# junka/ffpic

Measured on AMD Instinct MI355X. Metric: Mpixels/s decoded (dequant+IDCT+YUV->BGRA), 4K JPEG batch, higher is better.
Workload: dtype int16 -> int32 -> u8; 1 GPU; C3: 256 x 3840x2160 4:2:0 JPEG coefficient grids per GPU; images_total=256, images_this_rank=256, coded_size=3840x2160, subsampling=4:2:0, parallelism=image ranges over 1 GPU(s), no data-path collective, batch_close=one GPU: stream sync + own record, batch_complete=True

## Files before the change

ffpic_amd/csrc/ffhip_entropy.c:

```c
#include "ffpic_hip.h"
#include "ffhip_entropy_internal.h"

#include <pthread.h>
#include <stdio.h>
#include <stdlib.h>
#include <string.h>

static const uint8_t k_zigzag[64] = {0,  1,  8,  16, 9,  2,  3,  10, 17, 24, 32, 25, 18, 11, 4,  5,
                                     12, 19, 26, 33, 40, 48, 41, 34, 27, 20, 13, 6,  7,  14, 21, 28,
                                     35, 42, 49, 56, 57, 50, 43, 36, 29, 22, 15, 23, 30, 37, 44, 51,
                                     58, 59, 52, 45, 38, 31, 39, 46, 53, 60, 61, 54, 47, 55, 62, 63};

static int huff_build(struct huff *h, const uint8_t counts[16], const uint8_t *vals, int nvals)
{
    memset(h, 0, sizeof *h);
    int code = 0, k = 0;
    memcpy(h->vals, vals, (size_t)nvals);
    for (int len = 1; len <= 16; len++) {
        h->valptr[len] = k;
        h->mincode[len] = code;
        for (int i = 0; i < counts[len - 1]; i++, k++, code++) {
            if (k >= nvals) return -1;
            if (code >= (1 << len)) return -1;
            if (len <= LOOK) {
                int first = code << (LOOK - len), n = 1 << (LOOK - len);
                for (int j = 0; j < n; j++) h->look[first + j] = (uint16_t)((len << 8) | vals[k]);
            }
        }
        h->maxcode[len] = counts[len - 1] ? code - 1 : -1;
        code <<= 1;
    }
    h->maxcode[17] = 0x7fffffff;
    h->present = 1;
    for (int i = 0; i < (1 << LOOK); i++) {
        const unsigned e = h->look[i];
        const int len = (int)(e >> 8), run = (int)((e >> 4) & 15), mag = (int)(e & 15);
        if (!e || !mag || len + mag > LOOK) continue;
        int k = ((i << len) & ((1 << LOOK) - 1)) >> (LOOK - mag);
        if (k < (1 << (mag - 1))) k -= (1 << mag) - 1;
        if (k >= -128 && k <= 127) h->fast[i] = (int16_t)((k * 256) + (run * 16) + len + mag);
    }
    return 0;
}

struct bits {
    const uint8_t *p, *end;
    uint64_t acc;
    int n;
    int marker;
    int dry;
};

static inline void bits_fill(struct bits *b)
{
    if (!b->marker && b->end - b->p >= 8 && b->n <= 56) {
        uint64_t w;
        memcpy(&w, b->p, 8);
        w = __builtin_bswap64(w);
        const uint64_t x = ~w;
        if (!((x - 0x0101010101010101ULL) & ~x & 0x8080808080808080ULL)) {
            const int nb = (64 - b->n) >> 3;
            b->acc = nb == 8 ? w : (b->acc << (8 * nb)) | (w >> (64 - 8 * nb));
            b->p += nb;
            b->n += 8 * nb;
            return;
        }
    }
    while (b->n <= 56) {
        unsigned c = 0;
        int real = 0;
        if (!b->marker && b->p < b->end) {
            c = *b->p;
            if (c == 0xFF) {
                if (b->p + 1 < b->end && b->p[1] == 0) { b->p += 2; real = 1; }
                else { b->marker = 1; c = 0; }
            } else { b->p++; real = 1; }
        }
        b->dry += !real;
        b->acc = (b->acc << 8) | c;
        b->n += 8;
    }
}
static inline int bits_get(struct bits *b, int k)
{
    if (k == 0) return 0;
    if (b->n < k) bits_fill(b);
    b->n -= k;
    return (int)((b->acc >> b->n) & ((1u << k) - 1));
}
static inline int huff_decode(struct bits *b, const struct huff *h)
{
    if (b->n < 16) bits_fill(b);
    unsigned peek = (unsigned)((b->acc >> (b->n - LOOK)) & ((1u << LOOK) - 1));
    unsigned e = h->look[peek];
    if (e) { b->n -= (int)(e >> 8); return (int)(e & 0xff); }
    int code = (int)peek, len = LOOK;
    while (code > h->maxcode[len]) {
        if (++len > 16) return -1;
        code = (int)((b->acc >> (b->n - len)) & ((1u << len) - 1));
    }
    b->n -= len;
    return h->vals[(h->valptr[len] + code - h->mincode[len]) & 255];
}
static inline int extend(int v, int t) { return (t && v < (1 << (t - 1))) ? v - (1 << t) + 1 : v; }

static int parse_headers(const uint8_t *f, size_t len, struct jpeg_hdr *j)
{
    memset(j, 0, sizeof *j);
    for (int t = 0; t < 4; t++)
        for (int i = 0; i < 64; i++) j->quant[t][i] = 1;
    if (len < 4 || f[0] != 0xFF || f[1] != 0xD8) return FFHIP_EINVAL;
    size_t p = 2;
    int have_sof = 0;
    while (p + 4 <= len) {
        if (f[p] != 0xFF) return FFHIP_EINVAL;
        while (p < len && f[p] == 0xFF) p++;
        if (p >= len) return FFHIP_EINVAL;
        const int m = f[p++];
        if (m == 0xD9) return FFHIP_EINVAL;
        if (m == 0x01 || (m >= 0xD0 && m <= 0xD7)) continue;
        if (p + 2 > len) return FFHIP_EINVAL;
        const size_t L = ((size_t)f[p] << 8) | f[p + 1];
        if (L < 2 || p + L > len) return FFHIP_EINVAL;
        const uint8_t *s = f + p + 2;
        const size_t sl = L - 2;
        p += L;
        if (m == 0xDB) {
            size_t i = 0;
            while (i < sl) {
                const int prec = s[i] >> 4, id = s[i] & 15;
                i++;
                if (id > 3 || i + (size_t)64 * (prec + 1) > sl) return FFHIP_EINVAL;
                for (int k = 0; k < 64; k++, i += prec + 1)
                    j->quant[id][k_zigzag[k]] = prec ? (uint16_t)((s[i] << 8) | s[i + 1]) : s[i];
            }
        } else if (m == 0xC4) {
            size_t i = 0;
            while (i + 17 <= sl) {
                const int tc = s[i] >> 4, th = s[i] & 15;
                int n = 0;
                for (int k = 0; k < 16; k++) n += s[i + 1 + k];
                if (tc > 1 || th > 3 || n > 256 || i + 17 + (size_t)n > sl) return FFHIP_EINVAL;
                if (huff_build(tc ? &j->ac[th] : &j->dc[th], s + i + 1, s + i + 17, n)) return FFHIP_EINVAL;
                i += 17 + (size_t)n;
            }
        } else if (m == 0xC0 || m == 0xC1) {
            if (sl < 6 || s[0] != 8) return FFHIP_EINVAL;
            j->height = (s[1] << 8) | s[2];
            j->width = (s[3] << 8) | s[4];
            j->ncomp = s[5];
            if ((j->ncomp != 1 && j->ncomp != 3) || sl < (size_t)(6 + 3 * j->ncomp)) return FFHIP_EINVAL;
            if (j->width == 0 || j->height == 0) return FFHIP_EINVAL;
            for (int c = 0; c < j->ncomp; c++) {
                j->cid[c] = s[6 + 3 * c];
                j->h[c] = s[7 + 3 * c] >> 4;
                j->v[c] = s[7 + 3 * c] & 15;
                j->tq[c] = s[8 + 3 * c];
                if (j->tq[c] > 3) return FFHIP_EINVAL;
            }
            have_sof = 1;
        } else if (m == 0xC2 || (m >= 0xC5 && m <= 0xCF && m != 0xC8 && m != 0xCC)) {
            return FFHIP_EINVAL;
        } else if (m == 0xDD) {
            if (sl < 2) return FFHIP_EINVAL;
            j->restart = (s[0] << 8) | s[1];
        } else if (m == 0xDA) {
            if (!have_sof || sl < 1 || s[0] != j->ncomp || sl < (size_t)(4 + 2 * j->ncomp)) return FFHIP_EINVAL;
            for (int k = 0; k < j->ncomp; k++) {
                int c;
                for (c = 0; c < j->ncomp && j->cid[c] != s[1 + 2 * k]; c++) {}
                if (c == j->ncomp) return FFHIP_EINVAL;
                j->td[c] = s[2 + 2 * k] >> 4;
                j->ta[c] = s[2 + 2 * k] & 15;
                if (j->td[c] > 3 || j->ta[c] > 3 || !j->dc[j->td[c]].present || !j->ac[j->ta[c]].present) return FFHIP_EINVAL;
            }
            const uint8_t *t = s + 1 + 2 * j->ncomp;
            if (t[0] != 0 || t[1] != 63 || t[2] != 0) return FFHIP_EINVAL;
            j->scan = f + p;
            j->scan_len = len - p;
            break;
        }
    }
    if (!j->scan) return FFHIP_EINVAL;
    if (j->ncomp == 1) { j->h[0] = j->v[0] = 1; }
    if (j->h[0] < 1 || j->v[0] < 1 || j->h[0] * j->v[0] > 4) return FFHIP_EINVAL;
    for (int c = 1; c < j->ncomp; c++)
        if (j->h[c] != 1 || j->v[c] != 1) return FFHIP_EINVAL;
    return FFHIP_OK;
}

int ffhip_jpeg_parse(const uint8_t *file, size_t len, struct jpeg_hdr *j) { return parse_headers(file, len, j); }
int ffhip_jpeg_probe_restart(const uint8_t *file, size_t len)
{
    struct jpeg_hdr *j = malloc(sizeof *j);
    if (!j) return -1;
    const int r = parse_headers(file, len, j) ? -1 : j->restart;
    free(j);
    return r;
}

int ffhip_jpeg_probe(const uint8_t *file, size_t len, ffhip_jpeg_geom *geom, int *width, int *height)
{
    struct jpeg_hdr *j = malloc(sizeof *j);
    if (!j) return FFHIP_ENOMEM;
    int rc = file && geom ? parse_headers(file, len, j) : FFHIP_EINVAL;
    if (rc == FFHIP_OK) {
        geom->ncomp = j->ncomp;
        geom->h = j->h[0];
        geom->v = j->v[0];
        geom->mcu_cols = (j->width + 8 * j->h[0] - 1) / (8 * j->h[0]);
        geom->mcu_rows = (j->height + 8 * j->v[0] - 1) / (8 * j->v[0]);
        for (int c = 0; c < 3; c++) geom->qt_id[c] = c < j->ncomp ? j->tq[c] : 0;
        if (width) *width = j->width;
        if (height) *height = j->height;
    }
    free(j);
    return rc;
}

static int decode_mcus(const struct jpeg_hdr *j, int16_t *const planes[3], struct bits *b, long mcu, long count)
{
    int pred[3] = {0, 0, 0};
    for (int c = 0; c < j->ncomp; c++) {
        const size_t per = (size_t)j->h[c] * j->v[c] * 64;
        memset(planes[c] + (size_t)mcu * per, 0, (size_t)count * per * sizeof(int16_t));
    }
    for (const long end = mcu + count; mcu < end; mcu++) {
        for (int c = 0; c < j->ncomp; c++) {
            const struct huff *hd = &j->dc[j->td[c]], *ha = &j->ac[j->ta[c]];
            const int nb = j->h[c] * j->v[c];
            for (int k = 0; k < nb; k++) {
                int16_t *blk = planes[c] + (mcu * nb + k) * 64;
                const int t = huff_decode(b, hd);
                if (t < 0 || t > 11) return FFHIP_EINVAL;
                pred[c] += extend(bits_get(b, t), t);
                blk[0] = (int16_t)pred[c];
                for (int i = 1; i < 64;) {
                    if (b->n < 16) bits_fill(b);
                    const int f = ha->fast[(b->acc >> (b->n - LOOK)) & ((1u << LOOK) - 1)];
                    if (f) {
                        i += (f >> 4) & 15;
                        if (i > 63) return FFHIP_EINVAL;
                        b->n -= f & 15;
                        blk[k_zigzag[i++]] = (int16_t)(f >> 8);
                        continue;
                    }
                    const int rs = huff_decode(b, ha);
                    if (rs < 0) return FFHIP_EINVAL;
                    const int r = rs >> 4, s = rs & 15;
                    if (s == 0) {
                        if (r == 15) { i += 16; continue; }
                        break;
                    }
                    i += r;
                    if (i > 63) return FFHIP_EINVAL;
                    blk[k_zigzag[i]] = (int16_t)extend(bits_get(b, s), s);
                    i++;
                }
            }
        }
    }
    if (b->dry * 8 > b->n) return FFHIP_EINVAL;
    return FFHIP_OK;
}

struct interval_job {
    const struct jpeg_hdr *j;
    int16_t *planes[3];
    const size_t *seg;
    long n_seg, mcus, first, last;
    int rc;
};
static void *interval_worker(void *arg)
{
    struct interval_job *w = arg;
    w->rc = FFHIP_OK;
    for (long i = w->first; i < w->last && w->rc == FFHIP_OK; i++) {
        const uint8_t *p = w->j->scan + w->seg[i];
        const uint8_t *e = i + 1 < w->n_seg ? w->j->scan + w->seg[i + 1] - 2 : w->j->scan + w->j->scan_len;
        struct bits b = {p, e, 0, 0, 0, 0};
        const long mcu = i * w->j->restart, left = w->mcus - mcu;
        w->rc = decode_mcus(w->j, w->planes, &b, mcu, left < w->j->restart ? left : w->j->restart);
    }
    return NULL;
}

int ffhip_jpeg_entropy_decode_mt(const uint8_t *file, size_t len, const ffhip_jpeg_geom *expect, int16_t *coef_y,
                                 int16_t *coef_u, int16_t *coef_v, uint16_t *quant , int n_threads)
{
    struct jpeg_hdr *j = malloc(sizeof *j);
    if (!j) return FFHIP_ENOMEM;
    int rc = file && coef_y && quant ? parse_headers(file, len, j) : FFHIP_EINVAL;
    if (rc) { free(j); return rc; }
    const int mcu_cols = (j->width + 8 * j->h[0] - 1) / (8 * j->h[0]), mcu_rows = (j->height + 8 * j->v[0] - 1) / (8 * j->v[0]);
    if (expect && (expect->mcu_cols != mcu_cols || expect->mcu_rows != mcu_rows || expect->ncomp != j->ncomp ||
                   expect->h != j->h[0] || expect->v != j->v[0])) { free(j); return FFHIP_EINVAL; }
    if (j->ncomp == 3 && (!coef_u || !coef_v)) { free(j); return FFHIP_EINVAL; }
    memcpy(quant, j->quant, sizeof j->quant);
    const long mcus = (long)mcu_cols * mcu_rows;
    struct interval_job base = {j, {coef_y, coef_u, coef_v}, NULL, 1, mcus, 0, 1, FFHIP_OK};
    if (!j->restart) {
        struct bits b = {j->scan, j->scan + j->scan_len, 0, 0, 0, 0};
        rc = decode_mcus(j, base.planes, &b, 0, mcus);
        free(j);
        return rc;
    }
    const long n_seg = (mcus + j->restart - 1) / j->restart;
    size_t *seg = malloc((size_t)n_seg * sizeof *seg);
    if (!seg) { free(j); return FFHIP_ENOMEM; }
    long found = 1;
    seg[0] = 0;
    for (size_t q = 0; q + 1 < j->scan_len && found < n_seg; q++)
        if (j->scan[q] == 0xFF && j->scan[q + 1] >= 0xD0 && j->scan[q + 1] <= 0xD7) { seg[found++] = q + 2; q++; }
    if (found != n_seg) { free(seg); free(j); return FFHIP_EINVAL; }
    base.seg = seg;
    base.n_seg = n_seg;
    if (n_threads < 1) n_threads = 1;
    if (n_threads > n_seg) n_threads = (int)n_seg;
    if (n_threads > 64) n_threads = 64;
    struct interval_job jobs[64];
    pthread_t tid[64];
    int started[64] = {0};
    for (int t = 0; t < n_threads; t++) {
        jobs[t] = base;
        jobs[t].first = n_seg * t / n_threads;
        jobs[t].last = n_seg * (t + 1) / n_threads;
        if (t) started[t] = pthread_create(&tid[t], NULL, interval_worker, &jobs[t]) == 0;
    }
    interval_worker(&jobs[0]);
    rc = jobs[0].rc;
    for (int t = 1; t < n_threads; t++) {
        if (started[t]) pthread_join(tid[t], NULL);
        else interval_worker(&jobs[t]);
        if (rc == FFHIP_OK) rc = jobs[t].rc;
    }
    free(seg);
    free(j);
    return rc;
}

int ffhip_jpeg_entropy_decode(const uint8_t *file, size_t len, const ffhip_jpeg_geom *expect, int16_t *coef_y,
                              int16_t *coef_u, int16_t *coef_v, uint16_t *quant )
{
    return ffhip_jpeg_entropy_decode_mt(file, len, expect, coef_y, coef_u, coef_v, quant, 1);
}

struct batch_job {
    const uint8_t *const *files;
    const size_t *lens;
    const ffhip_jpeg_geom *g;
    int first, last;
    int16_t *y, *u, *v;
    uint16_t *quant;
    int *status;
};
static void blank_picture(int16_t *y, int16_t *u, int16_t *v, uint16_t *quant, size_t yb, size_t cb)
{
    memset(y, 0, yb * sizeof(int16_t));
    if (u) memset(u, 0, cb * sizeof(int16_t));
    if (v) memset(v, 0, cb * sizeof(int16_t));
    for (int i = 0; i < 256; i++) quant[i] = 1;
}
static void *batch_worker(void *arg)
{
    struct batch_job *jb = arg;
    const size_t mcus = (size_t)jb->g->mcu_cols * jb->g->mcu_rows, yb = mcus * jb->g->h * jb->g->v * 64, cb = mcus * 64;
    for (int i = jb->first; i < jb->last; i++) {
        jb->status[i] = ffhip_jpeg_entropy_decode(jb->files[i], jb->lens[i], jb->g, jb->y + i * yb, jb->u ? jb->u + i * cb : NULL,
                                                  jb->v ? jb->v + i * cb : NULL, jb->quant + (size_t)i * 256);
        if (jb->status[i]) blank_picture(jb->y + i * yb, jb->u ? jb->u + i * cb : NULL, jb->v ? jb->v + i * cb : NULL, jb->quant + (size_t)i * 256, yb, cb);
    }
    return NULL;
}

int ffhip_jpeg_entropy_batch(const uint8_t *const *files, const size_t *lens, int n, int n_threads,
                             const ffhip_jpeg_geom *geom, int16_t *coef_y, int16_t *coef_u, int16_t *coef_v,
                             uint16_t *quant, int *status)
{
    if (n < 0 || !geom || (n > 0 && (!files || !lens || !coef_y || !quant || !status))) return FFHIP_EINVAL;
    if (n == 0) return FFHIP_OK;
    if (n_threads < 1) n_threads = 1;
    if (n_threads >= 2 * n) {
        const size_t mcus = (size_t)geom->mcu_cols * geom->mcu_rows, yb = mcus * geom->h * geom->v * 64, cb = mcus * 64;
        int first_err = FFHIP_OK;
        for (int i = 0; i < n; i++) {
            status[i] = ffhip_jpeg_entropy_decode_mt(files[i], lens[i], geom, coef_y + (size_t)i * yb, coef_u ? coef_u + (size_t)i * cb : NULL,
                                                     coef_v ? coef_v + (size_t)i * cb : NULL, quant + (size_t)i * 256, n_threads);
            if (status[i]) blank_picture(coef_y + (size_t)i * yb, coef_u ? coef_u + (size_t)i * cb : NULL, coef_v ? coef_v + (size_t)i * cb : NULL, quant + (size_t)i * 256, yb, cb);
            if (status[i] && !first_err) first_err = status[i];
        }
        return first_err;
    }
    if (n_threads > n) n_threads = n;
    if (n_threads > 256) n_threads = 256;
    struct batch_job jobs[256];
    pthread_t tid[256];
    int started[256] = {0};
    for (int t = 0; t < n_threads; t++) {
        jobs[t] = (struct batch_job){files, lens, geom, (int)((long)n * t / n_threads), (int)((long)n * (t + 1) / n_threads),
                                     coef_y, coef_u, coef_v, quant, status};
        if (t) started[t] = pthread_create(&tid[t], NULL, batch_worker, &jobs[t]) == 0;
    }
    batch_worker(&jobs[0]);
    for (int t = 1; t < n_threads; t++) {
        if (started[t]) pthread_join(tid[t], NULL);
        else batch_worker(&jobs[t]);
    }
    for (int i = 0; i < n; i++)
        if (status[i]) return status[i];
    return FFHIP_OK;
}

int ffhip_bmp_write(const char *path, const uint8_t *bgra, int width, int height, int64_t pitch)
{
    if (!path || !bgra || width <= 0 || height <= 0 || pitch < (int64_t)width * 4) return FFHIP_EINVAL;
    FILE *f = fopen(path, "wb");
    if (!f) return FFHIP_EIO;
    uint8_t h[54] = {0};
    const uint32_t img = (uint32_t)width * (uint32_t)height * 4u, size = 54u + img;
    const int32_t neg_h = -height;
#define PUT32(o, v) do { uint32_t v__ = (uint32_t)(v); h[o] = v__ & 255; h[(o) + 1] = (v__ >> 8) & 255; h[(o) + 2] = (v__ >> 16) & 255; h[(o) + 3] = v__ >> 24; } while (0)
    h[0] = 'B'; h[1] = 'M';
    PUT32(2, size); PUT32(10, 0x36); PUT32(14, 0x28); PUT32(18, width); PUT32(22, neg_h);
    h[26] = 1; h[28] = 32;
    PUT32(34, img); PUT32(38, 0x60); PUT32(42, 0x60); PUT32(46, 2);
#undef PUT32
    int ok = fwrite(h, 54, 1, f) == 1;
    for (int y = 0; ok && y < height; y++) ok = fwrite(bgra + (size_t)y * (size_t)pitch, (size_t)width * 4, 1, f) == 1;
    ok = (fclose(f) == 0) && ok;
    return ok ? FFHIP_OK : FFHIP_EIO;
}
```

ffpic_amd/csrc/ffhip_entropy_internal.h:

```cpp
#ifndef FFHIP_ENTROPY_INTERNAL_H
#define FFHIP_ENTROPY_INTERNAL_H

#include <stddef.h>
#include <stdint.h>

#ifdef __cplusplus
extern "C" {
#endif

#define LOOK 9
struct huff {
    uint16_t look[1 << LOOK];
    int32_t maxcode[18];
    int32_t valptr[17], mincode[17];
    uint8_t vals[256];
    int present;
    int16_t fast[1 << LOOK];
};

struct jpeg_hdr {
    int width, height, ncomp, restart;
    int h[3], v[3], tq[3], td[3], ta[3], cid[3];
    uint16_t quant[4][64];
    struct huff dc[4], ac[4];
    const uint8_t *scan;
    size_t scan_len;
};

int ffhip_jpeg_parse(const uint8_t *file, size_t len, struct jpeg_hdr *j);
int ffhip_jpeg_probe_restart(const uint8_t *file, size_t len);

#ifdef __cplusplus
}
#endif
#endif
```

ffpic_amd/csrc/ffhip_huff_gpu.hip:

```cpp
#include "ffhip_internal.h"
#include <chrono>
#if defined(__SSE2__)
#include <emmintrin.h>
#endif
#include "ffhip_entropy_internal.h"

#include <stddef.h>
#include <stdlib.h>
#include <string.h>

#include <vector>
#include <memory>
#include <new>

struct HuffImage {
    uint32_t scan_off, scan_len;
    uint32_t seg_base, n_seg;
    uint32_t restart, mcus;
    uint32_t mcu_base;
    uint32_t ncomp, nb[3];
    uint32_t tab_dc[3], tab_ac[3];
};

struct HuffArgs {
    const uint8_t *scan;
    const struct huff *tabs;
    const uint16_t *lut;
    const HuffImage *images;
    const uint32_t *seg;
    const u32x2 *work;
    int16_t *plane[3];
    int *status;
    uint32_t n_work;
};

__device__ static const uint8_t kZigzag[64] = {0,  1,  8,  16, 9,  2,  3,  10, 17, 24, 32, 25, 18, 11, 4,  5,
                                               12, 19, 26, 33, 40, 48, 41, 34, 27, 20, 13, 6,  7,  14, 21, 28,
                                               35, 42, 49, 56, 57, 50, 43, 36, 29, 22, 15, 23, 30, 37, 44, 51,
                                               58, 59, 52, 45, 38, 31, 39, 46, 53, 60, 61, 54, 47, 55, 62, 63};

#define LUT_GROUPS 8
#define LUT_NO_CODE 0x5000u
#define LUT_WORDS (512 + 128 * LUT_GROUPS)

template <int RING_DW, int REFILL_EVERY>
__global__ __launch_bounds__(256) void k_jpeg_huff(HuffArgs a)
{
    __shared__ uint8_t zz[64];
    __shared__ uint16_t lt[6][LUT_WORDS];
    __shared__ uint32_t ring[4][RING_DW][64];
    const uint32_t lane = threadIdx.x & 63, wv = threadIdx.x >> 6;
    if (threadIdx.x < 64) zz[threadIdx.x] = kZigzag[threadIdx.x];
    const uint32_t gid0 = blockIdx.x * 256;
    const uint32_t img0 = a.work[gid0].x;
    const HuffImage im0 = a.images[img0];
    for (int t = 0; t < 3; t++) {
        const u32x4 *sd = (const u32x4 *)(a.lut + (size_t)im0.tab_dc[t] * LUT_WORDS), *sa = (const u32x4 *)(a.lut + (size_t)im0.tab_ac[t] * LUT_WORDS);
        for (int i = (int)threadIdx.x; i < LUT_WORDS / 8; i += 256) {
            ((u32x4 *)lt[t])[i] = sd[i];
            ((u32x4 *)lt[3 + t])[i] = sa[i];
        }
    }
    __syncthreads();
    const uint32_t gid = gid0 + wv * 64 + lane;
    const bool exists = gid < a.n_work;
    const u32x2 w = a.work[exists ? gid : gid0];
    const HuffImage im = a.images[w.x];
    bool in_lds = true;
    for (int t = 0; t < 3; t++) in_lds = in_lds && im.tab_dc[t] == im0.tab_dc[t] && im.tab_ac[t] == im0.tab_ac[t];
    const uint32_t start = im.scan_off + a.seg[im.seg_base + w.y];
    const u32x4 *src = (const u32x4 *)(a.scan + (start & ~15u));
    uint32_t rd = (start & 15u) >> 2, wr = 0;
    const uint32_t dw_end = (im.scan_off + a.seg[im.seg_base + w.y + 1] - (start & ~15u)) >> 2;
    uint32_t mcu = w.y * im.restart;
    const uint32_t mcu_end = mcu + im.restart < im.mcus ? mcu + im.restart : im.mcus;
    __shared__ uint32_t slotrec[4][8][64];
    __shared__ int predv[4][3][64];
    __shared__ unsigned long long planeb[4][3][64];
    uint32_t nbt = 0;
#pragma unroll
    for (int c = 0; c < 3; c++) {
        const unsigned long long pb = a.plane[c] ? (unsigned long long)(uintptr_t)(a.plane[c] + (size_t)im.mcu_base * im.nb[c] * 64) : 0ull;
        planeb[wv][c][lane] = pb;
        predv[wv][c][lane] = 0;
        for (uint32_t kb0 = 0; kb0 < im.nb[c] && nbt < 8; kb0++)
            slotrec[wv][nbt++][lane] = (uint32_t)c | (kb0 << 2) | (im.nb[c] << 5) | ((im.tab_dc[c] & 0xfffu) << 8) | ((im.tab_ac[c] & 0xfffu) << 20);
    }
    unsigned long long acc = 0;
    int n = 0;
    bool active = exists && mcu < mcu_end, bad = false;
    uint32_t slot = 0, k = 0, rec = slotrec[wv][0][lane];
    int16_t *blk = (int16_t *)(uintptr_t)planeb[wv][0][lane] + (size_t)mcu * im.nb[0] * 64;
    int pred_cur = 0;
    auto refill = [&]() {
        while (__builtin_amdgcn_ballot_w64(wr + 4 <= rd + RING_DW)) {
            if (wr + 4 <= rd + RING_DW) {
                u32x4 v = {0u, 0u, 0u, 0u};
                if (wr < dw_end) v = src[wr >> 2];
#pragma unroll
                for (int j = 0; j < 4; j++) ring[wv][(wr + j) & (RING_DW - 1)][lane] = wr + j < dw_end ? v[j] : 0u;
                wr += 4;
            }
        }
    };
    refill();
    for (int i = 0; i < 2; i++) {
        const uint32_t d = ring[wv][rd & (RING_DW - 1)][lane];
        acc = (acc << 32) | __builtin_bswap32(d);
        rd++;
    }
    n = 64;
    for (uint32_t iter = 1; __builtin_amdgcn_ballot_w64(active); iter++) {
        if ((iter & (REFILL_EVERY - 1)) == 0) refill();
        const uint32_t nextdw = ring[wv][rd & (RING_DW - 1)][lane];
        if (active) {
            const bool dc = k == 0;
            const uint32_t c = rec & 3u;
            const unsigned top = (unsigned)(acc >> 32);
            const unsigned peek = top >> (32 - LOOK);
            const uint32_t tix = dc ? (rec >> 8) & 0xfffu : rec >> 20;
            unsigned e;
            if (in_lds) {
                const uint16_t *l = lt[dc ? c : 3 + c];
                e = l[peek];
                if (e & 0x8000u) e = l[512 + ((e & 0xffu) << 7) + ((top >> (32 - 16)) & 127u)];
            } else {
                const uint16_t *l = a.lut + (size_t)tix * LUT_WORDS;
                e = l[peek];
                if (e & 0x8000u) e = l[512 + ((e & 0xffu) << 7) + ((top >> (32 - 16)) & 127u)];
            }
            int sym = (int)(e & 0xff), len = (int)((e >> 8) & 31u);
            bad |= (e & 0x4000u) != 0;
            if (!e) {
                const struct huff *T = a.tabs + tix;
                int code = (int)peek;
                len = LOOK;
                while (len < 17 && code > T->maxcode[len]) {
                    len++;
                    code = (int)(top >> (32 - len));
                }
                if (len > 16) { bad = true; len = 16; }
                sym = T->vals[(T->valptr[len] + code - T->mincode[len]) & 255];
            }
            acc <<= len;
            const int s = dc ? sym : (sym & 15), r = dc ? 0 : (sym >> 4);
            const bool skip = !dc && s == 0;
            k += skip ? (r == 15 ? 16u : 64u) : (uint32_t)r;
            const unsigned vb = (unsigned)((acc >> 33) >> (31 - s));
            acc <<= s;
            n -= len + s;
            const int lim = (1 << s) >> 1;
            int v = (int)vb < lim ? (int)vb - (1 << s) + 1 : (int)vb;
            pred_cur += dc ? v : 0;
            v = dc ? pred_cur : v;
            bad |= (dc && s > 11) || (!skip && k > 63);
            if (!skip && k <= 63) blk[zz[k]] = (int16_t)v;
            k += skip ? 0u : 1u;
            if (k >= 64) {
                k = 0;
                slot++;
                const bool wrap = slot == nbt;
                slot = wrap ? 0u : slot;
                mcu += wrap ? 1u : 0u;
                rec = slotrec[wv][slot][lane];
                const uint32_t c2 = rec & 3u, nbc = (rec >> 5) & 7u, kb = (rec >> 2) & 7u;
                predv[wv][c][lane] = pred_cur;
                pred_cur = predv[wv][c2][lane];
                blk = (int16_t *)(uintptr_t)planeb[wv][c2][lane] + (size_t)(mcu * nbc + kb) * 64;
                if (mcu >= mcu_end) active = false;
            }
            bad |= rd > dw_end + 2;
#ifdef HUFF_DEBUG
            if (rd > dw_end + 2) printf("lane %u img %u seg %u: rd %u lim %u start %u mcu %u/%u k %u n %d\n", gid, w.x, w.y, rd, dw_end, start, mcu, mcu_end, k, n);
#endif
            if (bad) active = false;
            if (n <= 32) {
                acc |= (unsigned long long)__builtin_bswap32(nextdw) << (32 - n);
                n += 32;
                rd++;
            }
        }
    }
    if (bad) a.status[w.x] = FFHIP_EINVAL;
}

namespace {
uint32_t stage_scan(uint8_t *dst, const uint8_t *src, const uint8_t *end, uint32_t *seg, uint32_t n_seg, size_t *clean_len, uint32_t *raw = nullptr)
{
    uint8_t *d = dst;
    uint32_t k = 0;
    seg[0] = 0;
    for (;;) {
#if defined(__SSE2__)
        const __m128i ff = _mm_set1_epi8((char)0xFF);
        while (src + 16 <= end) {
            const __m128i v = _mm_loadu_si128((const __m128i *)src);
            const unsigned m = (unsigned)_mm_movemask_epi8(_mm_cmpeq_epi8(v, ff));
            _mm_storeu_si128((__m128i *)d, v);
            if (m) {
                const int c = __builtin_ctz(m);
                src += c;
                d += c;
                break;
            }
            src += 16;
            d += 16;
        }
#endif
        while (src < end && *src != 0xFF) *d++ = *src++;
        if (src + 1 >= end) break;
        const uint8_t b = src[1];
        if (b == 0) { *d++ = 0xFF; src += 2; continue; }
        if (b < 0xD0 || b > 0xD7 || k + 1 >= n_seg) break;
        {
            const size_t len = (size_t)(d - dst) - seg[k], padded = ((len + 3) & ~(size_t)3) + 4;
            memset(d, 0, padded - len);
            d = dst + seg[k] + padded;
            if (raw) raw[k] = (uint32_t)len;
            seg[++k] = (uint32_t)(d - dst);
            src += 2;
        }
    }
    {
        const size_t len = (size_t)(d - dst) - seg[k], padded = ((len + 3) & ~(size_t)3) + 4;
        memset(d, 0, padded - len);
        d = dst + seg[k] + padded;
        if (raw) raw[k] = (uint32_t)len;
    }
    *clean_len = (size_t)(d - dst);
    return k + 1;
}

void build_lut(const struct huff &h, uint16_t *out)
{
    memset(out, 0, LUT_WORDS * sizeof(uint16_t));
    memcpy(out, h.look, 512 * sizeof(uint16_t));
    int groups = 0;
    bool complete = true;
    for (int len = LOOK + 1; len <= 16; len++) {
        if (h.maxcode[len] < 0) continue;
        for (int code = h.mincode[len]; code <= h.maxcode[len]; code++) {
            const int idx = h.valptr[len] + code - h.mincode[len];
            if (idx < 0 || idx > 255 || code >= (1 << len)) return;
            const int prefix = code >> (len - LOOK);
            if (out[prefix] && !(out[prefix] & 0x8000)) return;
            if (!out[prefix]) {
                if (groups == LUT_GROUPS) { complete = false; continue; }
                out[prefix] = (uint16_t)(0x8000 | groups++);
            }
            const int g = out[prefix] & 0xff;
            const int rest = (code << (16 - len)) & 127, cnt = 1 << (16 - len);
            for (int k = 0; k < cnt; k++) out[512 + 128 * g + rest + k] = (uint16_t)((len << 8) | h.vals[idx]);
        }
    }
    if (complete)
        for (int i = 0; i < 512 + 128 * groups; i++)
            if (!out[i]) out[i] = LUT_NO_CODE;
}
}

extern "C" int ffhip_jpeg_stage_scan_test(uint8_t *dst, const uint8_t *src, size_t len, uint32_t *seg, uint32_t n_seg, size_t *clean_len)
{
    if (!dst || !src || !seg || !clean_len || n_seg == 0) return FFHIP_EINVAL;
    return (int)stage_scan(dst, src, src + len, seg, n_seg, clean_len);
}

extern "C" int ffhip_jpeg_stage_scan_raw_test(uint8_t *dst, const uint8_t *src, size_t len, uint32_t *seg, uint32_t n_seg, size_t *clean_len, uint32_t *raw)
{
    if (!dst || !src || !seg || !clean_len || !raw || n_seg == 0) return FFHIP_EINVAL;
    return (int)stage_scan(dst, src, src + len, seg, n_seg, clean_len, raw);
}
extern "C" int ffhip_jpeg_lut_test(const uint8_t *file, size_t len, int which, uint16_t *out)
{
    if (!file || !out || which < 0 || which > 7) return FFHIP_EINVAL;
    std::unique_ptr<struct jpeg_hdr> j(new (std::nothrow) struct jpeg_hdr);
    if (!j) return FFHIP_ENOMEM;
    if (ffhip_jpeg_parse(file, len, j.get())) return FFHIP_EINVAL;
    const struct huff &h = which < 4 ? j->dc[which] : j->ac[which - 4];
    if (!h.present) return FFHIP_EINVAL;
    build_lut(h, out);
    return FFHIP_OK;
}

static thread_local double g_huff_times[8] = {0, 0, 0, 0, 0, 0, 0, 0};
static uint32_t sync_sub_bits(unsigned long long bits, unsigned long long mcus)
{
    const char *b = FFHIP_ENV("FFHIP_JPEG_SYNC_BITS");
    const long sb = b ? atol(b) : bits <= 1024 * mcus ? 2048 : bits <= 2048 * mcus ? 4096 : 8192;
    return (uint32_t)(sb < 128 ? 128 : sb > 65536 ? 65536 : sb);
}
extern "C" int ffhip_debug_huff_times(double out[8])
{
    if (!out) return FFHIP_EINVAL;
    for (int k = 0; k < 8; k++) out[k] = g_huff_times[k];
    return FFHIP_OK;
}

struct SyncSeg {
    uint32_t pic;
    uint32_t scan_off, clean_len;
    uint32_t raw_len;
    uint32_t mcu0, mcus;
};
struct SyncJob {
    uint8_t *dev;
    size_t o_tabs, o_l12, o_status;
    int n, part;
    void *stream;
    const HuffImage *images;
    const SyncSeg *segs;
    size_t n_segs;
    int16_t *plane[3];
    uint32_t rounds_used;
    uint32_t n_tasks;
    int reran;
    uint32_t rounds;
    uint32_t sub_bits;
};
static int huff_sync_enqueue(SyncJob &job, void *stream, uint32_t **h_cnt);
static int huff_sync_finish(SyncJob &job, void *stream, uint32_t *h_cnt, int *status);

namespace {
typedef std::chrono::steady_clock::time_point HuffTime;
HuffTime huff_now() { return std::chrono::steady_clock::now(); }
long us(HuffTime a, HuffTime b) { return (long)std::chrono::duration_cast<std::chrono::microseconds>(b - a).count(); }
struct HuffLayout { size_t o_tabs, o_l12, o_img, o_seg, o_work, o_status, o_quant, total; };
HuffLayout huff_layout(size_t scan_total, size_t n_tabs, size_t n, size_t seg_total)
{
    HuffLayout L;
    size_t at = scan_total + 16;
    auto take = [&](size_t bytes) { const size_t o = at; at = (at + bytes + 15) & ~(size_t)15; return o; };
    L.o_tabs = take(n_tabs * sizeof(struct huff));
    L.o_l12 = take(n_tabs * LUT_WORDS * 2);
    L.o_img = take(n * sizeof(HuffImage));
    L.o_seg = take((seg_total + n) * 4);
    L.o_work = take(seg_total * 8);
    L.o_status = take(n * 4);
    L.o_quant = take(n * 512);
    L.total = at;
    return L;
}
struct HuffCall {
    const uint8_t *const *files;
    const size_t *lens;
    int n, n_threads;
    const ffhip_jpeg_geom *geom, *geoms;
    int16_t *d_coef_y, *d_coef_u, *d_coef_v;
    uint16_t *d_quant;
    int *status;
    hipStream_t st;
    const FfhipHuffThen *then;
    std::vector<uint32_t> pic_mcus, mcu_base;
    struct jpeg_hdr *hdr;
    std::vector<std::vector<uint32_t>> segs, raws;
    uint32_t sub_bits;
    std::vector<HuffImage> images;
    std::vector<const struct huff *> uniq;
    size_t scan_total, seg_total;
    HuffLayout L;
    uint8_t *stage, *dev;
    hipStream_t up, second;
    hipEvent_t fork, join, *part_ev, time_ev[2];
    std::vector<ffhip_jpeg_item> then_items;
    bool times;
    HuffTime T0, T1, T2, T3, T4;
    long staging_us, tables_us;
};

#define HUFF_TRY(call) do { if ((call) != hipSuccess) return FFHIP_EIO; } while (0)
int huff_first_status(const HuffCall &c) { for (int i = 0; i < c.n; i++) if (c.status[i]) return c.status[i]; return FFHIP_OK; }
int huff_check(HuffCall &c)
{
    const ffhip_jpeg_geom *geom = c.geom;
    if (geom->ncomp == 3 && (!c.d_coef_u || !c.d_coef_v)) return FFHIP_EINVAL;
    c.n_threads = c.n_threads < 1 ? 1 : c.n_threads > 64 ? 64 : c.n_threads;
    if (geom->mcu_cols <= 0 || geom->mcu_rows <= 0 || geom->h < 1 || geom->v < 1 || geom->h * geom->v > 4 ||
        (geom->ncomp != 1 && geom->ncomp != 3)) return FFHIP_EINVAL;
    c.pic_mcus.resize((size_t)c.n);
    c.mcu_base.resize((size_t)c.n + 1);
    size_t sum = 0;
    for (int i = 0; i < c.n; i++) {
        const ffhip_jpeg_geom *gi = c.geoms ? &c.geoms[i] : geom;
        if (c.geoms && (gi->ncomp != geom->ncomp || gi->h != geom->h || gi->v != geom->v || gi->mcu_cols <= 0 || gi->mcu_rows <= 0)) return FFHIP_EINVAL;
        c.pic_mcus[(size_t)i] = (uint32_t)((size_t)gi->mcu_cols * gi->mcu_rows);
        c.mcu_base[(size_t)i] = (uint32_t)sum;
        sum += c.pic_mcus[(size_t)i];
        if (sum > 0xffffffffu) return FFHIP_EINVAL;
    }
    c.mcu_base[(size_t)c.n] = (uint32_t)sum;
    return FFHIP_OK;
}
int huff_parse_headers(HuffCall &c)
{
    c.hdr = ffhip_huff_hdr_records((size_t)c.n);
    if (!c.hdr) return FFHIP_ENOMEM;
    c.segs.resize((size_t)c.n);
    c.raws.resize((size_t)c.n);
    ffhip_parallel_for(c.n, c.n_threads, [&c](int i) {
        struct jpeg_hdr &j = c.hdr[(size_t)i];
        c.status[i] = ffhip_jpeg_parse(c.files[i], c.lens[i], &j);
        if (c.status[i]) return;
        const int mc = (j.width + 8 * j.h[0] - 1) / (8 * j.h[0]), mr = (j.height + 8 * j.v[0] - 1) / (8 * j.v[0]);
        const ffhip_jpeg_geom *gi = c.geoms ? &c.geoms[i] : c.geom;
        const size_t mcus = c.pic_mcus[(size_t)i];
        if (mc != gi->mcu_cols || mr != gi->mcu_rows || j.ncomp != gi->ncomp || j.h[0] != gi->h || j.v[0] != gi->v ||
            j.scan_len > 0x7fffffffu) {
            c.status[i] = FFHIP_EINVAL;
            return;
        }
        if (!j.restart) j.restart = (int)mcus;
        c.segs[(size_t)i].assign((size_t)((mcus + j.restart - 1) / j.restart) + 1, 0u);
        c.raws[(size_t)i].assign(c.segs[(size_t)i].size(), 0u);
    });
    return huff_first_status(c);
}
bool huff_choose_subsequences(HuffCall &c)
{
    const char *sy = FFHIP_ENV("FFHIP_JPEG_SYNC");
    unsigned long long batch_bits = 0, n_int = 0;
    for (int i = 0; i < c.n; i++) batch_bits += 8ull * c.hdr[(size_t)i].scan_len;
    c.sub_bits = sync_sub_bits(batch_bits, (unsigned long long)c.mcu_base[(size_t)c.n]);
    if (sy && (sy[0] == '0' || sy[0] == '1')) return sy[0] == '1';
    for (int i = 0; i < c.n; i++) n_int += c.segs[(size_t)i].size() - 1;
    return batch_bits > 2ull * c.sub_bits * n_int;
}
uint32_t huff_table_id(std::vector<const struct huff *> &uniq, const struct huff *t)
{
    for (size_t u = uniq.size(); u-- > 0;)
        if (uniq[u] == t || !memcmp(&uniq[u]->maxcode, &t->maxcode, offsetof(struct huff, fast) - offsetof(struct huff, maxcode))) return (uint32_t)u;
    uniq.push_back(t);
    return (uint32_t)(uniq.size() - 1);
}
int huff_lay_out(HuffCall &c)
{
    c.images.resize((size_t)c.n);
    c.scan_total = c.seg_total = 0;
    for (int i = 0; i < c.n; i++) {
        const struct jpeg_hdr &j = c.hdr[(size_t)i];
        HuffImage &im = c.images[(size_t)i];
        im.scan_off = (uint32_t)c.scan_total;
        im.scan_len = (uint32_t)j.scan_len;
        im.restart = (uint32_t)j.restart;
        im.mcus = c.pic_mcus[(size_t)i];
        im.mcu_base = c.mcu_base[(size_t)i];
        im.ncomp = (uint32_t)j.ncomp;
        im.seg_base = (uint32_t)c.seg_total;
        im.n_seg = (uint32_t)c.segs[(size_t)i].size() - 1;
        for (int k = 0; k < 3; k++) {
            im.nb[k] = k < j.ncomp ? (uint32_t)(j.h[k] * j.v[k]) : 0;
            im.tab_dc[k] = huff_table_id(c.uniq, &j.dc[k < j.ncomp ? j.td[k] : j.td[0]]);
            im.tab_ac[k] = huff_table_id(c.uniq, &j.ac[k < j.ncomp ? j.ta[k] : j.ta[0]]);
        }
        c.scan_total += (j.scan_len + 8 * (size_t)im.n_seg + 64 + 15) & ~(size_t)15;
        c.seg_total += im.n_seg;
        im.seg_base += (uint32_t)i;
        if (c.scan_total > 0x7fffffffu) return FFHIP_EINVAL;
    }
    if (!ffhip_have_device()) return FFHIP_ENODEV;
    if (c.uniq.size() > 4095) return FFHIP_EINVAL;
    c.L = huff_layout(c.scan_total, c.uniq.size(), (size_t)c.n, c.seg_total);
    c.stage = ffhip_pinned_scratch(SCRATCH_HUFF, c.st, c.L.total + 64);
    if (!c.stage) return FFHIP_ENOMEM;
    c.T2 = huff_now();
    c.dev = (uint8_t *)ffhip_scratch(SCRATCH_HUFF, c.st, (c.L.total + 3) / 4);
    return c.dev ? FFHIP_OK : FFHIP_ENOMEM;
}
int huff_clear_planes(HuffCall &c)
{
    const size_t total_mcus = c.mcu_base[(size_t)c.n], yb = total_mcus * c.geom->h * c.geom->v * 64;
    FFHIP_CHECK(hipMemsetAsync(c.d_coef_y, 0, yb * 2, c.st), FFHIP_EIO);
    if (c.geom->ncomp != 3) return FFHIP_OK;
    FFHIP_CHECK(hipMemsetAsync(c.d_coef_u, 0, total_mcus * 128, c.st), FFHIP_EIO);
    FFHIP_CHECK(hipMemsetAsync(c.d_coef_v, 0, total_mcus * 128, c.st), FFHIP_EIO);
    return FFHIP_OK;
}
void huff_stage_pictures(HuffCall &c, int lo, int hi, bool lists)
{
    ffhip_parallel_for(hi - lo, c.n_threads, [&c, lo, lists](int i_rel) {
        const int i = lo + i_rel;
        const struct jpeg_hdr &j = c.hdr[(size_t)i];
        const HuffImage &im = c.images[(size_t)i];
        uint8_t *dst = c.stage + im.scan_off;
        std::vector<uint32_t> &sgv = c.segs[(size_t)i];
        size_t off = 0;
        if (stage_scan(dst, j.scan, j.scan + j.scan_len, sgv.data(), im.n_seg, &off, c.raws[(size_t)i].data()) != im.n_seg) c.status[i] = FFHIP_EINVAL;
        memset(dst + off, 0, 16);
        sgv[im.n_seg] = (uint32_t)off;
        if (!lists) return;
        uint32_t *sg = (uint32_t *)(c.stage + c.L.o_seg) + im.seg_base;
        u32x2 *wk = (u32x2 *)(c.stage + c.L.o_work) + (im.seg_base - (uint32_t)i);
        for (uint32_t k = 0; k < im.n_seg; k++) {
            sg[k] = sgv[k];
            wk[k].x = (uint32_t)i;
            wk[k].y = k;
        }
        sg[im.n_seg] = (uint32_t)off;
        memcpy(c.stage + c.L.o_quant + (size_t)i * 512, j.quant, 512);
    });
}
int huff_part_lo(const HuffCall &c, int n_parts, int part) { return (int)((long long)c.n * part / n_parts); }
size_t huff_scan_end(const HuffCall &c, int hi) { return hi < c.n ? c.images[(size_t)hi].scan_off : c.scan_total; }

int huff_tail_up(HuffCall &c)
{
    const HuffTime Ta = huff_now();
    memset(c.stage + c.scan_total, 0, 16);
    ffhip_parallel_for((int)c.uniq.size(), c.n_threads, [&c](int u) {
        ((struct huff *)(c.stage + c.L.o_tabs))[u] = *c.uniq[(size_t)u];
        build_lut(*c.uniq[(size_t)u], (uint16_t *)(c.stage + c.L.o_l12) + (size_t)u * LUT_WORDS);
    });
    memcpy(c.stage + c.L.o_img, c.images.data(), c.images.size() * sizeof(HuffImage));
    memset(c.stage + c.L.o_status, 0, (size_t)c.n * 4);
    c.tables_us = us(Ta, huff_now());
    FFHIP_CHECK(hipMemcpyAsync(c.dev + c.scan_total, c.stage + c.scan_total, c.L.total - c.scan_total, hipMemcpyHostToDevice, c.st), FFHIP_EIO);
    FFHIP_CHECK(hipMemcpyAsync(c.d_quant, c.dev + c.L.o_quant, (size_t)c.n * 512, hipMemcpyDeviceToDevice, c.st), FFHIP_EIO);
    return FFHIP_OK;
}
int huff_reconstruct(HuffCall &c, int lo, int hi, void *on, int part)
{
    const FfhipHuffThen *then = c.then;
    if (!then->items) {
        const size_t mcus = c.pic_mcus[0];
        return ffhip_jpeg_recon_batch(c.geom, hi - lo, c.d_coef_y + (size_t)lo * mcus * c.geom->h * c.geom->v * 64, c.d_coef_u ? c.d_coef_u + (size_t)lo * mcus * 64 : nullptr,
                                      c.d_coef_v ? c.d_coef_v + (size_t)lo * mcus * 64 : nullptr, c.d_quant + (size_t)lo * 256, 256,
                                      then->bgra + (int64_t)lo * then->image_stride, then->pitch, then->image_stride, nullptr, 0, on);
    }
    c.then_items.assign(then->items + lo, then->items + hi);
    for (int i = lo; i < hi; i++) jpeg_item_planes(&c.then_items[(size_t)(i - lo)], c.d_coef_y, c.d_coef_u, c.d_coef_v, c.d_quant, c.mcu_base[(size_t)i], (size_t)i);
    return jpeg_recon_items_by_rule(c.then_items.data(), then->rule.at(lo), hi - lo, on, part);
}
int huff_collect(HuffCall &c)
{
    HUFF_TRY(hipMemcpyAsync(c.stage + c.L.o_status, c.dev + c.L.o_status, (size_t)c.n * 4, hipMemcpyDeviceToHost, c.st));
    const HuffTime T5 = huff_now();
    HUFF_TRY(hipStreamSynchronize(c.st));
    const HuffTime T6 = huff_now();
    if (c.times) {
        fprintf(stderr, "huff staging: header parse %ld us, layout %ld us, unstuff + markers (uploads enqueued by parts) %ld us, tables %ld us (%d files, %zu bytes, %d threads)\n", us(c.T0, c.T1), us(c.T1, c.T2), c.staging_us, c.tables_us, c.n, c.L.total, c.n_threads);
        fprintf(stderr, "huff device: enqueue %ld us, wait for uploads + clears + kernel %ld us\n", us(c.T3, T5), us(T5, T6));
    }
    float kms = 0.0f;
    if (hipEventElapsedTime(&kms, c.time_ev[0], c.time_ev[1]) != hipSuccess) { (void)hipGetLastError(); kms = 0.0f; }
    g_huff_times[0] = (double)us(c.T0, c.T1); g_huff_times[1] = (double)us(c.T1, c.T2); g_huff_times[2] = (double)c.staging_us; g_huff_times[3] = (double)c.tables_us;
    g_huff_times[4] = (double)us(c.T4, T5); g_huff_times[5] = (double)us(T5, T6); g_huff_times[6] = (double)kms * 1e3; g_huff_times[7] = (double)us(c.T0, T6);
    memcpy(c.status, c.stage + c.L.o_status, (size_t)c.n * 4);
    return FFHIP_OK;
}
int huff_decode_intervals(HuffCall &c)
{
    const int n_parts = c.n >= 32 ? 4 : 1;
    for (int part = 0; part < n_parts; part++) {
        const int lo = huff_part_lo(c, n_parts, part), hi = huff_part_lo(c, n_parts, part + 1);
        const size_t b0 = huff_scan_end(c, lo), b1 = huff_scan_end(c, hi);
        huff_stage_pictures(c, lo, hi, true);
        HUFF_TRY(hipMemcpyAsync(c.dev + b0, c.stage + b0, b1 - b0, hipMemcpyHostToDevice, c.st));
    }
    if (huff_first_status(c)) return huff_first_status(c);
    c.T3 = huff_now();
    c.staging_us = us(c.T2, c.T3);
    const int rc = huff_tail_up(c);
    if (rc) return rc;
    c.T4 = huff_now();
    HuffArgs a;
    a.scan = c.dev;
    a.tabs = (const struct huff *)(c.dev + c.L.o_tabs);
    a.lut = (const uint16_t *)(c.dev + c.L.o_l12);
    a.images = (const HuffImage *)(c.dev + c.L.o_img);
    a.seg = (const uint32_t *)(c.dev + c.L.o_seg);
    a.work = (const u32x2 *)(c.dev + c.L.o_work);
    a.plane[0] = c.d_coef_y; a.plane[1] = c.d_coef_u; a.plane[2] = c.d_coef_v;
    a.status = (int *)(c.dev + c.L.o_status);
    a.n_work = (uint32_t)c.seg_total;
    (void)hipEventRecord(c.time_ev[0], c.st);
    {
        int cus = 256, device = 0;
        if (hipGetDevice(&device) == hipSuccess) (void)hipDeviceGetAttribute(&cus, hipDeviceAttributeMultiprocessorCount, device);
        const unsigned wgs = (a.n_work + 255) / 256;
        const char *fr = FFHIP_ENV("FFHIP_HUFF_RING");
        if (fr ? atoi(fr) == 16 : wgs > 2u * (unsigned)cus) hipLaunchKernelGGL((k_jpeg_huff<16, 8>), dim3(wgs), dim3(256), 0, c.st, a);
        else hipLaunchKernelGGL((k_jpeg_huff<32, 16>), dim3(wgs), dim3(256), 0, c.st, a);
    }
    HUFF_TRY(hipGetLastError());
    (void)hipEventRecord(c.time_ev[1], c.st);
    if (c.then) {
        const int rrc = huff_reconstruct(c, 0, c.n, c.st, 0);
        if (rrc) return rrc;
    }
    return huff_collect(c);
}
int huff_sync_part_count(const HuffCall &c)
{
    const int by_bytes = (int)((c.scan_total + (70u << 20)) / (140u << 20));
    int n_parts = c.n < 32 || c.scan_total < (16u << 20) ? 1 : by_bytes < 2 ? 2 : by_bytes > FFHIP_HUFF_PARTS ? FFHIP_HUFF_PARTS : by_bytes;
    const char *e = FFHIP_ENV("FFHIP_JPEG_SYNC_PARTS");
    if (e && atoi(e) >= 1) n_parts = atoi(e) > FFHIP_HUFF_PARTS ? FFHIP_HUFF_PARTS : atoi(e);
    return n_parts > c.n ? c.n : n_parts;
}
int huff_sync_job(const HuffCall &c, SyncJob &job, std::vector<SyncSeg> &segs, int part, int lo, int hi)
{
    job.sub_bits = c.sub_bits;
    job.dev = c.dev; job.o_tabs = c.L.o_tabs; job.o_l12 = c.L.o_l12; job.o_status = c.L.o_status + (size_t)lo * 4; job.n = hi - lo; job.part = part;
    job.images = c.images.data() + lo;
    segs.clear();
    for (int i = lo; i < hi; i++) {
        const HuffImage &im = c.images[(size_t)i];
        const std::vector<uint32_t> &sgv = c.segs[(size_t)i];
        if (c.status[i]) return c.status[i];
        for (uint32_t k = 0; k < im.n_seg; k++) {
            SyncSeg sg;
            sg.pic = (uint32_t)(i - lo);
            sg.scan_off = im.scan_off + sgv[k];
            sg.clean_len = sgv[k + 1] - sgv[k];
            sg.raw_len = c.raws[(size_t)i][k];
            sg.mcu0 = (uint32_t)((size_t)(c.mcu_base[(size_t)i] - c.mcu_base[(size_t)lo]) + (size_t)k * im.restart);
            const size_t left = im.mcus - (size_t)k * im.restart;
            sg.mcus = (uint32_t)(left < im.restart ? left : im.restart);
            segs.push_back(sg);
        }
    }
    job.segs = segs.data();
    job.n_segs = segs.size();
    const size_t base = c.mcu_base[(size_t)lo];
    job.plane[0] = c.d_coef_y + base * c.images[0].nb[0] * 64;
    job.plane[1] = c.d_coef_u ? c.d_coef_u + base * c.images[0].nb[1] * 64 : nullptr;
    job.plane[2] = c.d_coef_v ? c.d_coef_v + base * c.images[0].nb[2] * 64 : nullptr;
    return FFHIP_OK;
}
int huff_decode_subsequences(HuffCall &c)
{
    const int n_parts = huff_sync_part_count(c);
    SyncJob jobs[FFHIP_HUFF_PARTS];
    std::vector<SyncSeg> part_segs[FFHIP_HUFF_PARTS];
    uint32_t *h_cnt[FFHIP_HUFF_PARTS];
    for (int i = 0; i < c.n; i++) memcpy(c.stage + c.L.o_quant + (size_t)i * 512, c.hdr[(size_t)i].quant, 512);
    int rc = huff_tail_up(c);
    if (rc) return rc;
    (void)hipEventRecord(c.time_ev[0], c.st);
    const char *ss = FFHIP_ENV("FFHIP_JPEG_SYNC_STREAMS");
    const bool two_streams = n_parts > 1 && !(ss && ss[0] == '1');
    if (two_streams) {
        HUFF_TRY(hipEventRecord(c.fork, c.st));
        HUFF_TRY(hipStreamWaitEvent(c.second, c.fork, 0));
    }
    for (int part = 0; part < n_parts; part++) {
        const int lo = huff_part_lo(c, n_parts, part), hi = huff_part_lo(c, n_parts, part + 1);
        SyncJob &job = jobs[part];
        const size_t b0 = huff_scan_end(c, lo), b1 = huff_scan_end(c, hi);
        huff_stage_pictures(c, lo, hi, false);
        job.stream = two_streams && (part & 1) ? (void *)c.second : c.st;
        HUFF_TRY(hipMemcpyAsync(c.dev + b0, c.stage + b0, b1 - b0, hipMemcpyHostToDevice, c.up));
        HUFF_TRY(hipEventRecord(c.part_ev[part], c.up));
        HUFF_TRY(hipStreamWaitEvent((hipStream_t)job.stream, c.part_ev[part], 0));
        rc = huff_sync_job(c, job, part_segs[part], part, lo, hi);
        if (!rc) rc = huff_sync_enqueue(job, job.stream, &h_cnt[part]);
        if (!rc && c.then) rc = huff_reconstruct(c, lo, hi, job.stream, part);
        if (rc) return rc;
    }
    if (two_streams) {
        HUFF_TRY(hipEventRecord(c.join, c.second));
        HUFF_TRY(hipStreamWaitEvent(c.st, c.join, 0));
    }
    c.T3 = c.T4 = huff_now();
    c.staging_us = us(c.T2, c.T3) - c.tables_us;
    HUFF_TRY(hipGetLastError());
    (void)hipEventRecord(c.time_ev[1], c.st);
    rc = huff_collect(c);
    if (rc) return rc;
    for (int part = 0; part < n_parts; part++) {
        SyncJob &job = jobs[part];
        const int lo = huff_part_lo(c, n_parts, part);
        rc = huff_sync_finish(job, job.stream, h_cnt[part], c.status + lo);
        if (!rc && job.reran && c.then) {
            rc = huff_reconstruct(c, lo, lo + job.n, job.stream, part);
            if (!rc && job.stream != c.st && hipStreamSynchronize((hipStream_t)job.stream) != hipSuccess) rc = FFHIP_EIO;
        }
        if (rc) return rc;
        if (c.times) fprintf(stderr, "huff sync, part %d: %u subsequences of %u bits, %u rounds\n", part, job.n_tasks, job.sub_bits, job.rounds_used);
    }
    return FFHIP_OK;
}
}

int jpeg_entropy_batch_gpu_impl(const uint8_t *const *files, const size_t *lens, int n, int n_threads, const ffhip_jpeg_geom *geom,
                                const ffhip_jpeg_geom *geoms, int16_t *d_coef_y, int16_t *d_coef_u, int16_t *d_coef_v, uint16_t *d_quant,
                                int *status, void *stream, const FfhipHuffThen *then)
{
    if (n < 0 || !geom || (n > 0 && (!files || !lens || !d_coef_y || !d_quant || !status))) return FFHIP_EINVAL;
    if (n == 0) return FFHIP_OK;
    HuffCall c{files, lens, n, n_threads, geom, geoms, d_coef_y, d_coef_u, d_coef_v, d_quant, status, (hipStream_t)stream, then};
    int rc = huff_check(c);
    if (rc) return rc;
    c.times = FFHIP_ENV("FFHIP_HUFF_TIMES") != nullptr;
    c.T0 = huff_now();
    rc = huff_parse_headers(c);
    if (rc) return rc;
    const bool subsequences = huff_choose_subsequences(c);
    c.T1 = huff_now();
    rc = huff_lay_out(c);
    if (rc) return rc;
    rc = huff_clear_planes(c);
    if (rc) return rc;
    FfhipHuffStreams hs;
    if (ffhip_huff_streams_get(&hs) != FFHIP_OK) return FFHIP_EIO;
    c.up = (hipStream_t)hs.up; c.second = (hipStream_t)hs.c2;
    c.part_ev = (hipEvent_t *)hs.part_ev;
    c.fork = (hipEvent_t)hs.fork; c.join = (hipEvent_t)hs.join;
    c.time_ev[0] = (hipEvent_t)hs.time_ev[0]; c.time_ev[1] = (hipEvent_t)hs.time_ev[1];
    rc = subsequences ? huff_decode_subsequences(c) : huff_decode_intervals(c);
    if (rc) {
        (void)hipStreamSynchronize(c.up);
        (void)hipStreamSynchronize(c.second);
        (void)hipStreamSynchronize(c.st);
        (void)hipGetLastError();
        return rc;
    }
    return huff_first_status(c);
}
extern "C" int ffhip_jpeg_entropy_batch_gpu(const uint8_t *const *files, const size_t *lens, int n, int n_threads,
                                            const ffhip_jpeg_geom *geom, int16_t *d_coef_y, int16_t *d_coef_u, int16_t *d_coef_v,
                                            uint16_t *d_quant, int *status, void *stream)
{
    return jpeg_entropy_batch_gpu_impl(files, lens, n, n_threads, geom, nullptr, d_coef_y, d_coef_u, d_coef_v, d_quant, status, stream, nullptr);
}

#define SYNC_ROUNDS_MAX 32

struct SyncImage {
    uint32_t scan_off;
    uint32_t clean_len;
    uint32_t data_bits;
    uint32_t mcus, ncomp, nbt;
    uint32_t nb[3], tab_dc[3], tab_ac[3];
    uint32_t pic, mcu0;
};
struct SyncArgs {
    const uint8_t *scan;
    const struct huff *tabs;
    const uint16_t *lut;
    const SyncImage *images;
    const uint32_t *sub_base;
    unsigned long long *exit_;
    unsigned long long *used;
    u32x4 *sums;
    uint32_t *list;
    uint32_t *seg_of;
    uint32_t *cnt;
    uint32_t *end_pos;
    int16_t *plane[3];
    int *status;
    uint32_t n_tasks, n_images, round, last, sub_bits;
};

__device__ __forceinline__ uint32_t sync_picture_of(const SyncArgs &a, uint32_t t)
{
    return a.seg_of[t];
}
__global__ __launch_bounds__(256) void k_huff_sync_segs(SyncArgs a)
{
    const uint32_t p = blockIdx.x, t1 = a.sub_base[p + 1];
    for (uint32_t t = a.sub_base[p] + threadIdx.x; t < t1; t += 256) a.seg_of[t] = p;
}

#define LIST_THREADS 1024
__global__ __launch_bounds__(LIST_THREADS) void k_huff_sync_list(SyncArgs a)
{
    __shared__ uint32_t wcount[LIST_THREADS / 64], wbase[LIST_THREADS / 64];
    if (a.round >= 3 && a.cnt[a.round - 1] == 0) return;
    const uint32_t t = blockIdx.x * LIST_THREADS + threadIdx.x, lane = threadIdx.x & 63, wv = threadIdx.x >> 6;
    bool stale = false;
    if (t > 0 && t < a.n_tasks) stale = a.seg_of[t - 1] == a.seg_of[t] && a.exit_[t - 1] != a.used[t];
    const unsigned long long m = __builtin_amdgcn_ballot_w64(stale);
    if (lane == 0) wcount[wv] = (uint32_t)__builtin_popcountll(m);
    __syncthreads();
    if (threadIdx.x == 0) {
        uint32_t total = 0;
        for (int w = 0; w < LIST_THREADS / 64; w++) { wbase[w] = total; total += wcount[w]; }
        const uint32_t base = total ? atomicAdd(&a.cnt[a.round], total) : 0u;
        for (int w = 0; w < LIST_THREADS / 64; w++) wbase[w] += base;
    }
    __syncthreads();
    if (stale) a.list[wbase[wv] + (uint32_t)__builtin_popcountll(m & ((1ull << lane) - 1ull))] = t;
}

enum { SPAN_ALL = 0, SPAN_LIST = 1, SPAN_WRITE = 2 };
#define SPAN_THREADS 512
#define WRITE_THREADS 256
template <int MODE, int THREADS>
__global__ __launch_bounds__(THREADS) void k_huff_span(SyncArgs a)
{
    constexpr bool WRITE = MODE == SPAN_WRITE;
    constexpr int RING = 16, REFILL = 4, WAVES = THREADS / 64;
    constexpr uint32_t LUT_BYTES = LUT_WORDS * 2;
    __shared__ uint8_t zz[64];
    __shared__ uint16_t lt[6][LUT_WORDS];
    __shared__ uint32_t ring[WAVES][RING][64];
    __shared__ u32x4 stage[WRITE ? 4 : 1][WRITE ? THREADS : 1];
    const uint32_t lane = threadIdx.x & 63, wv = threadIdx.x >> 6;
    const uint32_t i0 = blockIdx.x * THREADS;
    uint32_t n_here = a.n_tasks;
    if (MODE == SPAN_LIST) {
        n_here = a.cnt[a.round];
        if (i0 >= n_here) return;
    }
    if (WRITE && a.cnt[a.last]) return;
    if (threadIdx.x < 64) zz[threadIdx.x] = kZigzag[threadIdx.x];
    const uint32_t t_first = MODE == SPAN_LIST ? a.list[i0] : i0;
    const uint32_t p0 = sync_picture_of(a, t_first);
    const SyncImage im0 = a.images[p0];
    for (int k2 = 0; k2 < 3; k2++) {
        const u32x4 *sd = (const u32x4 *)(a.lut + (size_t)im0.tab_dc[k2] * LUT_WORDS), *sa = (const u32x4 *)(a.lut + (size_t)im0.tab_ac[k2] * LUT_WORDS);
        for (int i = (int)threadIdx.x; i < LUT_WORDS / 8; i += THREADS) {
            ((u32x4 *)lt[k2])[i] = sd[i];
            ((u32x4 *)lt[3 + k2])[i] = sa[i];
        }
    }
    if (WRITE)
        for (int i = 0; i < 4; i++) stage[i][threadIdx.x] = u32x4{0u, 0u, 0u, 0u};
    uint32_t cpack = 0, kbpack = 0, nbpack = 0;
    {
        uint32_t s = 0;
        for (uint32_t c = 0; c < 3; c++) {
            nbpack |= im0.nb[c] << (3 * c);
            for (uint32_t kb0 = 0; kb0 < im0.nb[c] && s < 8; kb0++, s++) {
                cpack |= c << (2 * s);
                kbpack |= kb0 << (3 * s);
            }
        }
    }
    __syncthreads();
    const uint32_t idx = i0 + threadIdx.x;
    const bool exists = idx < n_here;
    const uint32_t t = exists ? (MODE == SPAN_LIST ? a.list[idx] : idx) : t_first;
    const uint32_t p = exists ? sync_picture_of(a, t) : p0;
    const SyncImage im = a.images[p];
    bool in_lds = true;
    for (int k2 = 0; k2 < 3; k2++) in_lds = in_lds && im.tab_dc[k2] == im0.tab_dc[k2] && im.tab_ac[k2] == im0.tab_ac[k2];
    const uint32_t ti = t - a.sub_base[p];
    const uint32_t total_bits = im.clean_len * 8u;
    uint32_t limit = (ti + 1) * a.sub_bits;
    limit = limit < total_bits ? limit : total_bits;
    unsigned long long entry = 0;
    if (ti > 0) {
        if (WRITE) entry = a.used[t];
        else if (a.round == 0) entry = (unsigned long long)(ti * a.sub_bits);
        else entry = __hip_atomic_load(&a.exit_[t - 1], __ATOMIC_RELAXED, __HIP_MEMORY_SCOPE_AGENT);
    }
    const bool fresh = !WRITE && exists && (a.round == 0 || entry != a.used[t]);
    bool active = WRITE ? exists : fresh;
    uint32_t pos = (uint32_t)entry, slot = (uint32_t)(entry >> 32) & 0xffu, k = (uint32_t)(entry >> 40) & 0xffu;
    if (pos >= limit) active = false;
    const uint32_t nbt = im.nbt, ncomp = im.ncomp;
    u32x4 sm = {0u, 0u, 0u, 0u};
    if (WRITE && exists) sm = a.sums[t];
    slot = slot < nbt ? slot : 0;
    k = k < 64 ? k : 0;
    const uint32_t total_blocks = im.mcus * nbt;
    uint32_t bidx = 0, mcu = 0, blocks = 0;
    bool bad = false;
    if (WRITE) {
        bidx = sm[0];
        mcu = bidx / nbt;
        if (active && bidx < total_blocks && bidx - mcu * nbt != slot) { bad = true; active = false; }
        if (bidx >= total_blocks) active = false;
        mcu += im.mcu0;
    }
    uint32_t c = (cpack >> (2 * slot)) & 3u;
    int pcur, pn1, pn2;
    {
        const int q0 = (int)sm[1], q1 = (int)sm[2], q2 = (int)sm[3];
        pcur = c == 0 ? q0 : c == 1 ? q1 : q2;
        pn1 = c == 0 ? q1 : c == 1 ? q2 : q0;
        pn2 = c == 0 ? q2 : c == 1 ? q0 : q1;
    }
    const uint32_t start = im.scan_off + ((pos >> 5) << 2);
    const u32x4 *src = (const u32x4 *)(a.scan + (start & ~15u));
    uint32_t rd = (start & 15u) >> 2, wr = 0;
    const uint32_t dw_end = (im.scan_off + im.clean_len - (start & ~15u) + 3) >> 2;
    uint32_t *const myring = &ring[wv][0][lane];
    u32x4 pend = {0u, 0u, 0u, 0u};
    bool has_pend = false;
    auto issue = [&]() {
        pend = u32x4{0u, 0u, 0u, 0u};
        if (wr < dw_end) pend = src[wr >> 2];
        has_pend = true;
    };
    auto commit = [&]() {
        uint32_t *d = myring + (wr & (RING - 1)) * 64;
        d[0] = pend[0]; d[64] = pend[1]; d[128] = pend[2]; d[192] = pend[3];
        wr += 4;
        has_pend = false;
    };
    while (__builtin_amdgcn_ballot_w64(wr + 4 <= rd + RING))
        if (wr + 4 <= rd + RING) { issue(); commit(); }
    uint32_t w0 = 0, w1;
    int sh;
    {
        const uint32_t b = pos & 31u;
        if (b) { w0 = __builtin_bswap32(myring[(rd & (RING - 1)) * 64]); rd++; }
        w1 = __builtin_bswap32(myring[(rd & (RING - 1)) * 64]);
        rd++;
        sh = b ? 32 - (int)b : 0;
    }
    int16_t *blk = nullptr;
    auto block_of = [&]() -> int16_t * {
        const uint32_t nbc = (nbpack >> (3 * c)) & 7u, kb = (kbpack >> (3 * slot)) & 7u;
        int16_t *base = c == 0 ? a.plane[0] : c == 1 ? a.plane[1] : a.plane[2];
        return base + (size_t)(mcu * nbc + kb) * 64;
    };
    if (WRITE) blk = block_of();
    uint32_t tb_dc = c * LUT_BYTES;
    uint32_t cmask = 0;
    bool staged = k == 0;
    auto flush_rows = [&]() {
#pragma unroll
        for (int row = 0; row < 4; row++)
            if (cmask & (0xffu << (8 * row))) {
                const u32x4 q = stage[row][threadIdx.x];
                stage[row][threadIdx.x] = u32x4{0u, 0u, 0u, 0u};
                *(u32x4 *)(blk + 8 * row) = q;
            }
        cmask = 0;
    };
    __builtin_amdgcn_s_waitcnt(0x0f70);
    auto run = [&](auto lds_only) {
        constexpr bool LDS_ONLY = decltype(lds_only)::value;
        uint32_t iter = 1;
        while (active) {
            if ((iter & (REFILL - 1)) == 0) {
                if (has_pend) commit();
                if (wr + 4 <= rd + RING) issue();
            }
            iter++;
            const uint32_t nextdw = myring[(rd & (RING - 1)) * 64];
            const uint32_t W = __builtin_amdgcn_alignbit(w0, w1, (uint32_t)sh);
            const bool dc = k == 0;
            unsigned e;
            if (LDS_ONLY || in_lds) {
                const uint16_t *l = (const uint16_t *)((const uint8_t *)lt + tb_dc + (dc ? 0u : 3u * LUT_BYTES));
                e = l[W >> (32 - LOOK)];
                if (e & 0x8000u) e = l[512 + ((e & 0xffu) << 7) + ((W >> 16) & 127u)];
            } else {
                const uint32_t tix = dc ? (c == 0 ? im.tab_dc[0] : c == 1 ? im.tab_dc[1] : im.tab_dc[2]) : (c == 0 ? im.tab_ac[0] : c == 1 ? im.tab_ac[1] : im.tab_ac[2]);
                const uint16_t *l = a.lut + (size_t)tix * LUT_WORDS;
                e = l[W >> (32 - LOOK)];
                if (e & 0x8000u) e = l[512 + ((e & 0xffu) << 7) + ((W >> 16) & 127u)];
            }
            uint32_t sym = e & 0xffu, len = (e >> 8) & 31u;
            if (WRITE) bad |= (e & 0x4000u) != 0;
            if (!e) {
                const uint32_t tix = dc ? (c == 0 ? im.tab_dc[0] : c == 1 ? im.tab_dc[1] : im.tab_dc[2]) : (c == 0 ? im.tab_ac[0] : c == 1 ? im.tab_ac[1] : im.tab_ac[2]);
                const struct huff *T = a.tabs + tix;
                int code = (int)(W >> (32 - LOOK)), ln = LOOK;
                while (ln < 17 && code > T->maxcode[ln]) {
                    ln++;
                    code = (int)(W >> (32 - ln));
                }
                if (ln > 16) { bad = bad || WRITE; ln = 16; code = T->mincode[16]; }
                sym = T->vals[(T->valptr[ln] + code - T->mincode[ln]) & 255];
                len = (uint32_t)ln;
                __builtin_amdgcn_s_waitcnt(0x0f70);
            }
            const uint32_t s = sym & 15u, r = dc ? 0u : sym >> 4;
            const bool skip = !dc && s == 0;
            const uint32_t used = len + s;
            const uint32_t vb = __builtin_amdgcn_ubfe(W, 32u - used, s);
            const uint32_t m1 = (1u << s) - 1u;
            const int v = (vb << 1) > m1 ? (int)vb : (int)vb - (int)m1;
            pcur += dc ? v : 0;
            k += skip ? (r == 15 ? 16u : 64u) : r;
            if (WRITE) {
                bad |= (dc && sym > 11) || (!skip && k > 63);
                if (!skip && k <= 63) {
                    const uint32_t nat = zz[k];
                    const int16_t val = (int16_t)(dc ? pcur : v);
                    if (staged && nat < 32) {
                        ((int16_t *)&stage[nat >> 3][threadIdx.x])[nat & 7u] = val;
                        cmask |= 1u << nat;
                    } else blk[nat] = val;
                }
            }
            k += skip ? 0u : 1u;
            pos += used;
            sh -= (int)used;
            if (sh < 0) {
                w0 = w1;
                w1 = __builtin_bswap32(nextdw);
                sh += 32;
                rd++;
            }
            if (k >= 64) {
                k = 0;
                blocks++;
                slot++;
                const bool wrap = slot == nbt;
                slot = wrap ? 0u : slot;
                const uint32_t c2 = (cpack >> (2 * slot)) & 3u;
                if (c2 != c) { const int q = pcur; pcur = pn1; pn1 = ncomp == 3 ? pn2 : q; pn2 = q; }
                c = c2;
                tb_dc = c * LUT_BYTES;
                if (WRITE) {
                    flush_rows();
                    staged = true;
                    bidx++;
                    mcu += wrap ? 1u : 0u;
                    blk = block_of();
                    if (bidx >= total_blocks) { active = false; a.end_pos[p] = pos; }
                }
            }
            if (pos >= limit || bad) active = false;
        }
    };
    if (__builtin_amdgcn_ballot_w64(!in_lds) == 0) run(std::true_type{});
    else run(std::false_type{});
    if (WRITE) {
        while (cmask) {
            const uint32_t nat = (uint32_t)__builtin_ctz(cmask);
            cmask &= cmask - 1u;
            blk[nat] = ((const int16_t *)&stage[nat >> 3][threadIdx.x])[nat & 7u];
        }
        if (bad) a.status[im.pic] = FFHIP_EINVAL;
        return;
    }
    if (fresh) {
        const int q0 = c == 0 ? pcur : c == 1 ? pn2 : pn1, q1 = c == 0 ? pn1 : c == 1 ? pcur : pn2, q2 = c == 0 ? pn2 : c == 1 ? pn1 : pcur;
        const unsigned long long ex = (unsigned long long)pos | ((unsigned long long)(slot | (k << 8)) << 32);
        __hip_atomic_store(&a.exit_[t], ex, __ATOMIC_RELAXED, __HIP_MEMORY_SCOPE_AGENT);
        a.used[t] = entry;
        u32x4 o;
        o[0] = blocks; o[1] = (uint32_t)q0; o[2] = (uint32_t)q1; o[3] = (uint32_t)q2;
        a.sums[t] = o;
    }
}

__global__ __launch_bounds__(256) void k_huff_sync_scan(SyncArgs a)
{
    __shared__ u32x4 wsum[4];
    const uint32_t p = blockIdx.x;
    if (a.cnt[a.last]) return;
    const SyncImage im = a.images[p];
    const uint32_t t0 = a.sub_base[p], t1 = a.sub_base[p + 1];
    const int lane = threadIdx.x & 63, w = threadIdx.x >> 6;
    u32x4 carry = {0u, 0u, 0u, 0u};
    for (uint32_t base = t0; base < t1; base += 256) {
        const uint32_t t = base + threadIdx.x;
        u32x4 v = {0u, 0u, 0u, 0u};
        if (t < t1) v = a.sums[t];
        u32x4 inc = v;
#pragma unroll
        for (int o = 1; o < 64; o <<= 1) {
#pragma unroll
            for (int q = 0; q < 4; q++) {
                const uint32_t u = (uint32_t)__shfl_up((int)inc[q], o, 64);
                if (lane >= o) inc[q] += u;
            }
        }
        if (lane == 63) wsum[w] = inc;
        __syncthreads();
        u32x4 before = carry, total = {0u, 0u, 0u, 0u};
        for (int q = 0; q < 4; q++) {
            if (q < w) before += wsum[q];
            total += wsum[q];
        }
        if (t < t1) a.sums[t] = before + inc - v;
        carry += total;
        __syncthreads();
    }
    if (threadIdx.x == 0 && carry[0] < im.mcus * im.nbt) a.status[im.pic] = FFHIP_EINVAL;
}

__global__ __launch_bounds__(256) void k_huff_sync_verdict(SyncArgs a)
{
    const uint32_t p = blockIdx.x * 256 + threadIdx.x;
    if (a.cnt[a.last] || p >= a.n_images) return;
    if (a.end_pos[p] > a.images[p].data_bits) a.status[a.images[p].pic] = FFHIP_EINVAL;
}

namespace {
struct SyncLayout { size_t o_img, o_sub, o_cnt, o_end, o_list, o_seg, o_sums, o_exit, o_used, words; };
SyncLayout sync_layout(size_t n, size_t tasks)
{
    SyncLayout L;
    size_t w = 0;
    auto take = [&](size_t words) { const size_t at = w; w += (words + 3) & ~(size_t)3; return at; };
    L.o_img = take(n * sizeof(SyncImage) / 4);
    L.o_sub = take(n + 1);
    L.o_cnt = take(SYNC_ROUNDS_MAX + 3);
    L.o_end = take(n);
    L.o_list = take(tasks);
    L.o_seg = take(tasks);
    L.o_sums = take(4 * tasks);
    L.o_exit = take(2 * tasks);
    L.o_used = take(2 * tasks);
    L.words = w;
    return L;
}
void sync_args(SyncArgs &a, const SyncJob &job, uint32_t *d, const SyncLayout &L)
{
    a.scan = job.dev;
    a.tabs = (const struct huff *)(job.dev + job.o_tabs);
    a.lut = (const uint16_t *)(job.dev + job.o_l12);
    a.images = (const SyncImage *)(d + L.o_img);
    a.sub_base = d + L.o_sub;
    a.exit_ = (unsigned long long *)(d + L.o_exit);
    a.used = (unsigned long long *)(d + L.o_used);
    a.sums = (u32x4 *)(d + L.o_sums);
    a.list = d + L.o_list;
    a.seg_of = d + L.o_seg;
    a.cnt = d + L.o_cnt;
    a.end_pos = d + L.o_end;
    for (int c = 0; c < 3; c++) a.plane[c] = job.plane[c];
    a.status = (int *)(job.dev + job.o_status);
    a.n_tasks = job.n_tasks;
    a.n_images = (uint32_t)job.n_segs;
    a.round = 0;
    a.last = job.rounds + 2;
    a.sub_bits = job.sub_bits;
}
uint32_t sync_tasks_of(uint32_t raw_len, uint32_t sub_bits)
{
    const uint64_t bits = (uint64_t)raw_len * 8;
    return bits ? (uint32_t)((bits + sub_bits - 1) / sub_bits) : 1u;
}
int sync_launch_rounds_and_passes(SyncArgs &a, const SyncJob &job, hipStream_t st)
{
    const unsigned wgs = (job.n_tasks + SPAN_THREADS - 1) / SPAN_THREADS, wgl = (job.n_tasks + LIST_THREADS - 1) / LIST_THREADS;
    for (uint32_t r = 2; r <= job.rounds + 2; r++) {
        a.round = r;
        hipLaunchKernelGGL(k_huff_sync_list, dim3(wgl), dim3(LIST_THREADS), 0, st, a);
        if (r < job.rounds + 2) hipLaunchKernelGGL((k_huff_span<SPAN_LIST, SPAN_THREADS>), dim3(wgs), dim3(SPAN_THREADS), 0, st, a);
    }
    hipLaunchKernelGGL(k_huff_sync_scan, dim3((unsigned)job.n_segs), dim3(256), 0, st, a);
    hipLaunchKernelGGL((k_huff_span<SPAN_WRITE, WRITE_THREADS>), dim3((job.n_tasks + WRITE_THREADS - 1) / WRITE_THREADS), dim3(WRITE_THREADS), 0, st, a);
    hipLaunchKernelGGL(k_huff_sync_verdict, dim3(((unsigned)job.n_segs + 255) / 256), dim3(256), 0, st, a);
    FFHIP_CHECK(hipGetLastError(), FFHIP_EIO);
    return FFHIP_OK;
}
}

static int huff_sync_enqueue(SyncJob &job, void *stream, uint32_t **h_cnt)
{
    static_assert(sizeof(SyncImage) % 4 == 0, "SyncImage is copied by words");
    hipStream_t st = (hipStream_t)stream;
    const size_t n = job.n_segs;
    {
        const char *e = FFHIP_ENV("FFHIP_JPEG_SYNC_ROUNDS");
        const int r = e ? atoi(e) : 10;
        job.rounds = (uint32_t)(r < 1 ? 1 : r > SYNC_ROUNDS_MAX ? SYNC_ROUNDS_MAX : r);
        if (job.sub_bits < 128 || job.sub_bits > 65536) return FFHIP_EINVAL;
    }
    uint64_t tasks = 0;
    for (size_t i = 0; i < n; i++) {
        if (job.segs[i].clean_len >= (1u << 28)) return FFHIP_EINVAL;
        tasks += sync_tasks_of(job.segs[i].raw_len, job.sub_bits);
    }
    if (tasks > 0x7fffff00u || n > 0x7fffff00u) return FFHIP_EINVAL;
    const SyncLayout L = sync_layout(n, (size_t)tasks);
    const size_t head = L.o_list;
    uint8_t *pin = ffhip_pinned_scratch(SCRATCH_HUFF_SYNC + job.part, stream, (head + SYNC_ROUNDS_MAX + 3) * 4);
    uint32_t *d = ffhip_scratch(SCRATCH_HUFF_SYNC + job.part, stream, L.words);
    if (!pin || !d) return FFHIP_ENOMEM;
    uint32_t *h = (uint32_t *)pin;
    SyncImage *si = (SyncImage *)(h + L.o_img);
    uint32_t t = 0;
    for (size_t i = 0; i < n; i++) {
        const SyncSeg &sg = job.segs[i];
        const HuffImage &im = job.images[sg.pic];
        SyncImage &s = si[i];
        s.scan_off = sg.scan_off;
        s.clean_len = sg.clean_len;
        s.data_bits = sg.raw_len * 8u;
        s.mcus = sg.mcus;
        s.pic = sg.pic;
        s.mcu0 = sg.mcu0;
        s.ncomp = im.ncomp;
        s.nbt = 0;
        for (int c = 0; c < 3; c++) { s.nb[c] = im.nb[c]; s.tab_dc[c] = im.tab_dc[c]; s.tab_ac[c] = im.tab_ac[c]; s.nbt += im.nb[c]; }
        if (s.nb[0] != si[0].nb[0] || s.nb[1] != si[0].nb[1] || s.nb[2] != si[0].nb[2]) return FFHIP_EINVAL;
        h[L.o_sub + i] = t;
        t += sync_tasks_of(sg.raw_len, job.sub_bits);
    }
    h[L.o_sub + n] = t;
    job.n_tasks = t;
    memset(h + L.o_cnt, 0, (L.o_end - L.o_cnt) * 4);
    memset(h + L.o_end, 0xff, (L.o_list - L.o_end) * 4);
    FFHIP_CHECK(hipMemcpyAsync(d, h, head * 4, hipMemcpyHostToDevice, st), FFHIP_EIO);
    SyncArgs a;
    sync_args(a, job, d, L);
    const unsigned wgs = (t + SPAN_THREADS - 1) / SPAN_THREADS;
    hipLaunchKernelGGL(k_huff_sync_segs, dim3((unsigned)n), dim3(256), 0, st, a);
    for (uint32_t r = 0; r < 2; r++) {
        a.round = r;
        hipLaunchKernelGGL((k_huff_span<SPAN_ALL, SPAN_THREADS>), dim3(wgs), dim3(SPAN_THREADS), 0, st, a);
    }
    const int rc = sync_launch_rounds_and_passes(a, job, st);
    if (rc) return rc;
    *h_cnt = h + head;
    FFHIP_CHECK(hipMemcpyAsync(*h_cnt, d + L.o_cnt, (SYNC_ROUNDS_MAX + 3) * 4, hipMemcpyDeviceToHost, st), FFHIP_EIO);
    return FFHIP_OK;
}

static int huff_sync_finish(SyncJob &job, void *stream, uint32_t *h_cnt, int *status)
{
    hipStream_t st = (hipStream_t)stream;
    const uint32_t last = job.rounds + 2;
    job.rounds_used = 2;
    job.reran = 0;
    for (uint32_t r = 2; r < last; r++) job.rounds_used += h_cnt[r] ? 1u : 0u;
    if (!h_cnt[last]) return FFHIP_OK;
    const size_t n = job.n_segs;
    const SyncLayout L = sync_layout(n, job.n_tasks);
    uint32_t *d = ffhip_scratch(SCRATCH_HUFF_SYNC + job.part, stream, L.words);
    if (!d) return FFHIP_ENOMEM;
    SyncArgs a;
    sync_args(a, job, d, L);
    uint32_t longest = 0;
    for (size_t i = 0; i < n; i++) {
        const uint32_t ti = sync_tasks_of(job.segs[i].raw_len, job.sub_bits);
        longest = ti > longest ? ti : longest;
    }
    for (uint32_t done = last;; done += job.rounds) {
        if (done > longest + last) return FFHIP_EIO;
        memset(h_cnt, 0, (SYNC_ROUNDS_MAX + 3) * 4);
        FFHIP_CHECK(hipMemcpyAsync(d + L.o_cnt, h_cnt, (SYNC_ROUNDS_MAX + 3) * 4, hipMemcpyHostToDevice, st), FFHIP_EIO);
        const int rc = sync_launch_rounds_and_passes(a, job, st);
        if (rc) return rc;
        FFHIP_CHECK(hipMemcpyAsync(h_cnt, d + L.o_cnt, (SYNC_ROUNDS_MAX + 3) * 4, hipMemcpyDeviceToHost, st), FFHIP_EIO);
        FFHIP_CHECK(hipStreamSynchronize(st), FFHIP_EIO);
        for (uint32_t r = 2; r < last; r++) job.rounds_used += h_cnt[r] ? 1u : 0u;
        if (!h_cnt[last]) break;
    }
    FFHIP_CHECK(hipMemcpy(status, job.dev + job.o_status, (size_t)job.n * 4, hipMemcpyDeviceToHost), FFHIP_EIO);
    job.reran = 1;
    return FFHIP_OK;
}
```

ffpic_amd/csrc/ffhip_internal.h:

```cpp
#ifndef FFHIP_INTERNAL_H
#define FFHIP_INTERNAL_H

#include <hip/hip_runtime.h>
#include <stdint.h>

#include <functional>
#include <map>
#include <mutex>
#include <thread>
#include <vector>

#include "ffpic_hip.h"

#define FFHIP_CHECK(expr, code)                    \
    do {                                           \
        hipError_t e__ = (expr);                   \
        if (e__ != hipSuccess) {                   \
            ffhip_note_hip_error((int)e__, #expr); \
            return (code);                         \
        }                                          \
    } while (0)

#ifdef __cplusplus
extern "C" {
#endif
void ffhip_note_hip_error(int hip_error, const char *what);
int ffhip_have_device(void);
uint32_t *ffhip_scratch(int kind, void *stream, size_t words);
uint8_t *ffhip_pinned_scratch(int kind, void *stream, size_t bytes);
uint8_t *ffhip_pinned_staging(int kind, void *stream, size_t bytes);
int ffhip_pinned_staged(int kind, void *stream);
int *ffhip_async_err_word(void);
void ffhip_release_caches(void);
struct ffhip_env_site { const char *name; int gen; const char *val; };
const char *ffhip_env_lookup(struct ffhip_env_site *site);
int ffhip_resident_waves(const void *kernel, int block_threads);
#ifdef __cplusplus
}
#endif

#define FFHIP_ASYNC_BAD_INPUT 4

#ifdef __cplusplus
#define FFHIP_ENV(NAME) ([]() -> const char * { static struct ffhip_env_site site = {NAME, -1, nullptr}; return ffhip_env_lookup(&site); }())
#endif

template <class F> void ffhip_parallel_for(int count, int n_threads, F f)
{
    if (n_threads > count) n_threads = count;
    if (n_threads <= 1) { for (int i = 0; i < count; i++) f(i); return; }
    std::vector<std::thread> pool;
    auto part = [&](int t) { for (int i = t; i < count; i += n_threads) f(i); };
    for (int t = 1; t < n_threads; t++) pool.emplace_back(part, t);
    part(0);
    for (auto &th : pool) th.join();
}

typedef unsigned int u32;
typedef u32 u32x2 __attribute__((ext_vector_type(2)));
typedef u32 u32x4 __attribute__((ext_vector_type(4)));
typedef short s16x2 __attribute__((ext_vector_type(2)));
typedef short s16x4 __attribute__((ext_vector_type(4)));

#ifdef __HIPCC__
#define FFHIP_AUX_SC1 16
__device__ __forceinline__ __amdgpu_buffer_rsrc_t ffhip_rsrc(const void *base, unsigned bytes)
{
    return __builtin_amdgcn_make_buffer_rsrc((void *)base, 0, (int)bytes, 0x00020000);
}
__device__ __forceinline__ int ffhip_load_u8_sc1(__amdgpu_buffer_rsrc_t r, int byte_off)
{
    return (int)(unsigned char)__builtin_amdgcn_raw_buffer_load_b8(r, byte_off, 0, FFHIP_AUX_SC1);
}
__device__ __forceinline__ int ffhip_load_s16_sc1(__amdgpu_buffer_rsrc_t r, int byte_off)
{
    return (int)(short)__builtin_amdgcn_raw_buffer_load_b16(r, byte_off, 0, FFHIP_AUX_SC1);
}
#endif

enum FfhipScratchKind {
    SCRATCH_VP8_PRED = 1,
    SCRATCH_VP8_LF = 2,
    SCRATCH_HEVC_INTRA = 3,
    SCRATCH_HUFF = 4,
    SCRATCH_FILES_DEV = 5,
    SCRATCH_JPEG_HOST = 6,
    SCRATCH_VP8_RETRY = 8,
    SCRATCH_VP8_FRAMES = 9,
    SCRATCH_HEVC_TILES_ONE = 25,
    SCRATCH_HUFF_SYNC = 30,
    SCRATCH_FILES_MIXED = 7,
    SCRATCH_JPEG_ITEMS = 40,
    SCRATCH_WEBP = 60,
    SCRATCH_VP8_ITEMS = 50,
    SCRATCH_TENSOR_ITEMS = 70,
    SCRATCH_TENSOR_BGRA = 71,
    SCRATCH_RESIZE_ITEMS = 72,
    SCRATCH_RESIZE_BGRA = 73,
    SCRATCH_ORIENT_ITEMS = 74,
    SCRATCH_ORIENT_BGRA = 75,
    SCRATCH_JPEG_SCALED = 80,
    SCRATCH_JPEG_LIBJPEG = 100,
    SCRATCH_HUFF_PROG = 90,
};

struct Vp8ResItem {
    const int16_t *levels;
    const uint8_t *info;
    int16_t *out;
    long long first;
    uint16_t quant[32];
};
struct Vp8CheckItem { const uint8_t *modes; long long first;  };
int vp8_residual_items_enqueue(const Vp8ResItem *d_items, int n, long long n_mb, uint32_t *d_wg_item, void *stream);
int vp8_check_modes_items_enqueue(const Vp8CheckItem *d_items, int n, long long n_records, uint32_t *ctrl, int *async_err, void *stream);

struct FfhipVp8Then { uint8_t *bgra; int pitch; int64_t image_stride; };

struct Vp8SideBySide {
    hipStream_t side;
    hipEvent_t fork;
    int *err_word;
    const uint32_t *pred_progress;
    int pshift;
    int pred_split;
};
int vp8_predict_recon_impl(int mbcols, int mbrows, int n_images, const uint8_t *h_modes, const uint8_t *d_modes, const int16_t *d_residual,
                           int64_t residual_stride, const int32_t *d_resmap, uint8_t *d_y, uint8_t *d_u, uint8_t *d_v, int64_t plane_stride_y,
                           int64_t plane_stride_uv, void *stream, Vp8SideBySide *sbs);
int vp8_loopfilter_impl(int mbcols, int mbrows, int n_images, int filter_type, const uint8_t *d_modes, const uint8_t *d_filters, uint8_t *d_y,
                        uint8_t *d_u, uint8_t *d_v, int64_t plane_stride_y, int64_t plane_stride_uv, void *stream, const Vp8SideBySide *sbs);
struct Vp8RowSwitches { int pshift, slack; int *async_err; };
Vp8RowSwitches vp8_row_switches(const char *mode, const Vp8SideBySide *sbs);
int vp8_levels_upload_and_launch(int scratch_kind, void *stream, const std::vector<std::vector<uint32_t>> &lists,
                                 const std::function<void(const uint32_t *work, int count)> &launch);
int vp8_predict_loopfilter_impl(int mbcols, int mbrows, int n_images, const uint8_t *h_modes, const uint8_t *d_modes, const int16_t *d_residual,
                                int64_t residual_stride, const int32_t *d_resmap, int filter_type, const uint8_t *d_filters, uint8_t *d_y,
                                uint8_t *d_u, uint8_t *d_v, int64_t plane_stride_y, int64_t plane_stride_uv, void *stream, const FfhipVp8Then *then);

struct JpegPixelRule {
    const int *denom;
    const ffhip_size *display;
    JpegPixelRule at(int lo) const { return {denom ? denom + lo : nullptr, display ? display + lo : nullptr}; }
};
struct FfhipHuffThen { uint8_t *bgra; int64_t pitch, image_stride; const ffhip_jpeg_item *items; JpegPixelRule rule; };
int jpeg_entropy_batch_gpu_impl(const uint8_t *const *files, const size_t *lens, int n, int n_threads, const ffhip_jpeg_geom *geom,
                                const ffhip_jpeg_geom *geoms, int16_t *d_coef_y, int16_t *d_coef_u, int16_t *d_coef_v, uint16_t *d_quant,
                                int *status, void *stream, const FfhipHuffThen *then);
int jpeg_progressive_batch_gpu_impl(const uint8_t *const *files, const size_t *lens, int n, int n_threads, const ffhip_jpeg_geom *geom,
                                    const ffhip_jpeg_geom *geoms, int16_t *d_coef_y, int16_t *d_coef_u, int16_t *d_coef_v, uint16_t *d_quant,
                                    int k_max, const int *k_maxes, int *status, void *stream, const FfhipHuffThen *then, int counts[4]);
#define JPEG_CLASSES 7
struct JpegChoices {
    int variant;
    int remap;
    int strips[JPEG_CLASSES], mps[JPEG_CLASSES], per_wave[JPEG_CLASSES];
};
JpegChoices jpeg_choices(void);
int jpeg_item_class(const JpegChoices &ch, const ffhip_jpeg_geom *g, const uint8_t *d_bgra, int64_t pitch);
int jpeg_geom_class(const ffhip_jpeg_geom *g);
int jpeg_scaled_item_class(const ffhip_jpeg_geom *g, int denom, const uint8_t *d_bgra, int64_t pitch);
bool jpeg_libjpeg_item_ok(const ffhip_jpeg_geom *g, int width, int height, const uint8_t *d_bgra, int64_t pitch);
int jpeg_recon_items_impl(const ffhip_jpeg_item *items, int n, void *stream, int slot);
int jpeg_recon_items_scaled_impl(const ffhip_jpeg_item *items, const int *denom, int n, void *stream, int slot);
int jpeg_recon_items_libjpeg_impl(const ffhip_jpeg_item *items, const ffhip_size *display, int n, void *stream, int slot);
int jpeg_recon_items_by_rule(const ffhip_jpeg_item *items, const JpegPixelRule &rule, int n, void *stream, int slot);
int jpeg_rule_item_class(const JpegChoices &ch, const JpegPixelRule &rule, int i, const ffhip_jpeg_geom *g, int w, int h, const uint8_t *d_bgra, int64_t pitch);
struct JpegProbed { ffhip_jpeg_geom geom; int width, height, progressive, status; };
JpegProbed jpeg_probe_file(const uint8_t *file, size_t len, unsigned flags);
int jpeg_decode_files_mixed(const uint8_t *const *files, const size_t *lens, int n, int n_threads, uint8_t *const *d_bgra, const int64_t *pitch,
                            const int *denom, unsigned flags, ffhip_jpeg_geom *geom_out, int *status, void *stream);
inline void jpeg_item_planes(ffhip_jpeg_item *it, const int16_t *y, const int16_t *u, const int16_t *v, const uint16_t *q, size_t mcu_base, size_t index)
{
    it->d_coef_y = y + mcu_base * it->geom.h * it->geom.v * 64;
    it->d_coef_u = u ? u + mcu_base * 64 : nullptr;
    it->d_coef_v = v ? v + mcu_base * 64 : nullptr;
    it->d_quant = q + index * 256;
}

struct FfhipVp8Retry {
    bool armed = false;
    int mbcols = 0, mbrows = 0, n_images = 0, filter_type = 0;
    std::vector<uint8_t> h_modes;
    const uint8_t *d_modes = nullptr, *d_filters = nullptr;
    const int16_t *d_residual = nullptr;
    int64_t residual_stride = 0, plane_y = 0, plane_uv = 0;
    const int32_t *d_resmap = nullptr;
    uint8_t *y = nullptr, *u = nullptr, *v = nullptr, *keep = nullptr;
    FfhipVp8Then then = {nullptr, 0, 0};
    int *err = nullptr;
    unsigned long long seq = 0;
};
struct FfhipTileGuard {
    std::mutex turn;
    unsigned parity = 0;
    bool recorded[2] = {false, false};
    hipEvent_t ev[2] = {nullptr, nullptr};
};
struct FfhipBuf { void *p = nullptr; size_t cap = 0; };
struct FfhipStreamState {
    std::map<int, FfhipBuf> scratch, pinned;
    std::map<int, hipEvent_t> staged;
    FfhipVp8Retry retry;
    unsigned long long vp8_seq = 0;
    FfhipTileGuard tiles;
};
extern std::mutex g_ffhip_state_mu;
FfhipStreamState *ffhip_stream_state(void *stream, bool make = true);
void ffhip_state_release(void);
void ffhip_pipeline_release(void);
int ffhip_vp8_side_by_side_retry(void *stream);
struct jpeg_hdr *ffhip_huff_hdr_records(size_t n);

struct FfhipSide { void *stream, *fork, *join, *mid; };
extern "C" int ffhip_side_stream_get(FfhipSide *out);
struct FfhipPipe { void *plan, *plan_done; };
extern "C" int ffhip_pipe_streams_get(FfhipPipe *out);

#define FFHIP_HUFF_PARTS 8
struct FfhipHuffStreams { void *up, *c2, *part_ev[FFHIP_HUFF_PARTS], *fork, *join, *time_ev[2]; };
extern "C" int ffhip_huff_streams_get(FfhipHuffStreams *out);

#define FFHIP_VP8_CTRL_TICKET_C 32
#define FFHIP_VP8_CTRL_ABORT 64
#define FFHIP_VP8_CTRL_HDR 128
#define FFHIP_VP8_LF_CTRL_ABORT 32
#define FFHIP_VP8_LF_CTRL_HDR 64

#endif
```

ffpic_amd/csrc/ffhip_state.hip:

```cpp
#include "ffhip_internal.h"
#include "ffhip_entropy_internal.h"

#include <stdlib.h>

#include <algorithm>
#include <memory>
#include <new>
#include <utility>

std::mutex g_ffhip_state_mu;

namespace {
std::map<std::pair<int, void *>, FfhipStreamState> g_streams;

void *grow(FfhipBuf &b, size_t n, size_t unit, size_t pad, bool pinned, void *stream)
{
    if (n <= b.cap) return b.p;
    if (b.p) {
        if (hipStreamSynchronize((hipStream_t)stream) != hipSuccess) return nullptr;
        (void)(pinned ? hipHostFree(b.p) : hipFree(b.p));
    }
    b = FfhipBuf();
    const size_t want = n + n / 4 + pad;
    if ((pinned ? hipHostMalloc(&b.p, want * unit, hipHostMallocDefault) : hipMalloc(&b.p, want * unit)) != hipSuccess) { b.p = nullptr; return nullptr; }
    b.cap = want;
    return b.p;
}
void release(FfhipStreamState &s)
{
    for (auto &e : s.scratch) (void)hipFree(e.second.p);
    for (auto &e : s.pinned) (void)hipHostFree(e.second.p);
    for (auto &e : s.staged) (void)hipEventDestroy(e.second);
    if (s.retry.err) (void)hipHostFree(s.retry.err);
    for (hipEvent_t e : s.tiles.ev)
        if (e) (void)hipEventDestroy(e);
}
}

FfhipStreamState *ffhip_stream_state(void *stream, bool make)
{
    int dev = -1;
    (void)hipGetDevice(&dev);
    const auto key = std::make_pair(dev, stream);
    if (make) return &g_streams[key];
    auto it = g_streams.find(key);
    return it == g_streams.end() ? nullptr : &it->second;
}

extern "C" uint32_t *ffhip_scratch(int kind, void *stream, size_t words)
{
    std::lock_guard<std::mutex> lock(g_ffhip_state_mu);
    return (uint32_t *)grow(ffhip_stream_state(stream)->scratch[kind], words, sizeof(uint32_t), 1024, false, stream);
}
extern "C" uint8_t *ffhip_pinned_scratch(int kind, void *stream, size_t bytes)
{
    std::lock_guard<std::mutex> lock(g_ffhip_state_mu);
    return (uint8_t *)grow(ffhip_stream_state(stream)->pinned[kind], bytes, 1, 4096, true, stream);
}

extern "C" uint8_t *ffhip_pinned_staging(int kind, void *stream, size_t bytes)
{
    hipEvent_t ev = nullptr;
    {
        std::lock_guard<std::mutex> lock(g_ffhip_state_mu);
        auto &m = ffhip_stream_state(stream)->staged;
        auto it = m.find(kind);
        if (it != m.end()) ev = it->second;
    }
    if (ev && hipEventSynchronize(ev) != hipSuccess) return nullptr;
    return ffhip_pinned_scratch(kind, stream, bytes);
}
extern "C" int ffhip_pinned_staged(int kind, void *stream)
{
    std::lock_guard<std::mutex> lock(g_ffhip_state_mu);
    hipEvent_t &ev = ffhip_stream_state(stream)->staged[kind];
    if (!ev && hipEventCreateWithFlags(&ev, hipEventDisableTiming) != hipSuccess) { ev = nullptr; return FFHIP_EIO; }
    return hipEventRecord(ev, (hipStream_t)stream) == hipSuccess ? FFHIP_OK : FFHIP_EIO;
}

extern "C" void ffhip_stream_destroy(void *s)
{
    if (!s) return;
    (void)hipStreamSynchronize((hipStream_t)s);
    {
        std::lock_guard<std::mutex> lock(g_ffhip_state_mu);
        for (auto it = g_streams.begin(); it != g_streams.end();) {
            if (it->first.second != s) { ++it; continue; }
            const int *err = it->second.retry.err;
            if (err && *(volatile const int *)err) {
                int *g = ffhip_async_err_word();
                if (g) *(volatile int *)g = *(volatile const int *)err;
            }
            release(it->second);
            it = g_streams.erase(it);
        }
    }
    (void)hipStreamDestroy((hipStream_t)s);
}

namespace {
template <int NS, int NE> struct Group {
    hipStream_t s[NS] = {};
    hipEvent_t ev[NE] = {};
    void release()
    {
        for (auto &x : s) { if (x) (void)hipStreamDestroy(x); x = nullptr; }
        for (auto &e : ev) { if (e) (void)hipEventDestroy(e); e = nullptr; }
    }
    bool make(bool top, int timed = NE)
    {
        if (s[0]) return true;
        int least = 0, greatest = 0;
        const char *pe = FFHIP_ENV("FFHIP_SIDE_PRIORITY");
        top = top && !(pe && atoi(pe) == 0);
        if (top && hipDeviceGetStreamPriorityRange(&least, &greatest) != hipSuccess) { (void)hipGetLastError(); greatest = 0; }
        bool ok = true;
        for (auto &x : s)
            ok = ok && (top ? hipStreamCreateWithPriority(&x, hipStreamNonBlocking, greatest) : hipStreamCreateWithFlags(&x, hipStreamNonBlocking)) == hipSuccess;
        for (int k = 0; k < NE; k++) ok = ok && hipEventCreateWithFlags(&ev[k], k < timed ? hipEventDisableTiming : hipEventDefault) == hipSuccess;
        if (!ok) { (void)hipGetLastError(); release(); }
        return ok;
    }
};
struct ThreadSet {
    Group<1, 3> side;
    Group<1, 1> pipe;
    Group<2, FFHIP_HUFF_PARTS + 4> huff;
    void release() { side.release(); pipe.release(); huff.release(); }
};
struct ThreadState;
std::vector<ThreadState *> g_threads;
struct ThreadState {
    std::map<int, ThreadSet> sets;
    std::unique_ptr<struct jpeg_hdr[]> hdr;
    size_t hdr_cap = 0;
    ThreadState() { std::lock_guard<std::mutex> l(g_ffhip_state_mu); g_threads.push_back(this); }
    ~ThreadState()
    {
        std::lock_guard<std::mutex> l(g_ffhip_state_mu);
        g_threads.erase(std::remove(g_threads.begin(), g_threads.end(), this), g_threads.end());
        for (auto &e : sets) e.second.release();
    }
};
ThreadState &this_thread() { static thread_local ThreadState t; return t; }
template <class G> G *thread_group(G ThreadSet::*which, bool top, int timed)
{
    ThreadState &ts = this_thread();
    int dev = -1;
    if (hipGetDevice(&dev) != hipSuccess) return nullptr;
    std::lock_guard<std::mutex> l(g_ffhip_state_mu);
    G &g = ts.sets[dev].*which;
    return g.make(top, timed) ? &g : nullptr;
}
}

extern "C" int ffhip_side_stream_get(FfhipSide *out)
{
    const auto *g = thread_group(&ThreadSet::side, true, 3);
    if (!g) return FFHIP_EIO;
    *out = {g->s[0], g->ev[0], g->ev[1], g->ev[2]};
    return FFHIP_OK;
}
extern "C" int ffhip_pipe_streams_get(FfhipPipe *out)
{
    const auto *g = thread_group(&ThreadSet::pipe, false, 1);
    if (!g) return FFHIP_EIO;
    *out = {g->s[0], g->ev[0]};
    return FFHIP_OK;
}
extern "C" int ffhip_huff_streams_get(FfhipHuffStreams *out)
{
    const auto *g = thread_group(&ThreadSet::huff, false, FFHIP_HUFF_PARTS + 2);
    if (!g) return FFHIP_EIO;
    out->up = g->s[0]; out->c2 = g->s[1];
    for (int k = 0; k < FFHIP_HUFF_PARTS; k++) out->part_ev[k] = g->ev[k];
    out->fork = g->ev[FFHIP_HUFF_PARTS]; out->join = g->ev[FFHIP_HUFF_PARTS + 1];
    out->time_ev[0] = g->ev[FFHIP_HUFF_PARTS + 2]; out->time_ev[1] = g->ev[FFHIP_HUFF_PARTS + 3];
    return FFHIP_OK;
}

struct jpeg_hdr *ffhip_huff_hdr_records(size_t n)
{
    ThreadState &t = this_thread();
    std::lock_guard<std::mutex> l(g_ffhip_state_mu);
    if (n > t.hdr_cap) {
        t.hdr.reset(new (std::nothrow) struct jpeg_hdr[n + n / 4]);
        t.hdr_cap = t.hdr ? n + n / 4 : 0;
    }
    return t.hdr.get();
}

void ffhip_state_release(void)
{
    ffhip_pipeline_release();
    std::lock_guard<std::mutex> l(g_ffhip_state_mu);
    for (auto &e : g_streams) release(e.second);
    g_streams.clear();
    for (ThreadState *t : g_threads) {
        for (auto &e : t->sets) e.second.release();
        t->sets.clear();
        t->hdr.reset();
        t->hdr_cap = 0;
    }
}
```

Baseline: 851,700 Mpixels/s.

## Defer Huffman table building and dedupe specs by digest across batch

Header parsing now stores raw Huffman specs (counts, values, digest) and no longer builds full lookup tables for every DHT segment. Tables are deduplicated across the batch with a hash-slot resolver, and only the unique ones are built, in parallel, into a persistent per-thread buffer. Per-image segment vectors are replaced by one flat reused array, and small per-call mallocs become stack objects. The aim is to cut host-side parse and layout cost in the batch path, at the price of added hashing logic and a hard cap on the number of unique tables.

```diff
diff --git a/ffpic_amd/csrc/ffhip_entropy.c b/ffpic_amd/csrc/ffhip_entropy.c
--- a/ffpic_amd/csrc/ffhip_entropy.c
+++ b/ffpic_amd/csrc/ffhip_entropy.c
@@ -6,13 +6,30 @@
 #include <stdlib.h>
 #include <string.h>
 
-static const uint8_t k_zigzag[64] = {0,  1,  8,  16, 9,  2,  3,  10, 17, 24, 32, 25, 18, 11, 4,  5,
-                                     12, 19, 26, 33, 40, 48, 41, 34, 27, 20, 13, 6,  7,  14, 21, 28,
-                                     35, 42, 49, 56, 57, 50, 43, 36, 29, 22, 15, 23, 30, 37, 44, 51,
-                                     58, 59, 52, 45, 38, 31, 39, 46, 53, 60, 61, 54, 47, 55, 62, 63};
-
-static int huff_build(struct huff *h, const uint8_t counts[16], const uint8_t *vals, int nvals)
-{
+const uint8_t ffhip_zigzag[64] = {0,  1,  8,  16, 9,  2,  3,  10, 17, 24, 32, 25, 18, 11, 4,  5,
+                                  12, 19, 26, 33, 40, 48, 41, 34, 27, 20, 13, 6,  7,  14, 21, 28,
+                                  35, 42, 49, 56, 57, 50, 43, 36, 29, 22, 15, 23, 30, 37, 44, 51,
+                                  58, 59, 52, 45, 38, 31, 39, 46, 53, 60, 61, 54, 47, 55, 62, 63};
+
+static int huff_spec_check(const uint8_t counts[16], int nvals)
+{
+    int code = 0, k = 0;
+    for (int len = 1; len <= 16; len++) {
+        const int c = counts[len - 1];
+        if (c) {
+            if (k + c > nvals) return -1;
+            if (code + c > (1 << len)) return -1;
+        }
+        k += c;
+        code = (code + c) << 1;
+    }
+    return 0;
+}
+
+int ffhip_huff_build(struct huff *h, const struct huff_spec *s)
+{
+    const uint8_t *counts = s->counts, *vals = s->vals;
+    const int nvals = s->n;
     memset(h, 0, sizeof *h);
     int code = 0, k = 0;
     memcpy(h->vals, vals, (size_t)nvals);
@@ -43,66 +60,27 @@
     return 0;
 }
 
-struct bits {
-    const uint8_t *p, *end;
-    uint64_t acc;
-    int n;
-    int marker;
-    int dry;
-};
-
-static inline void bits_fill(struct bits *b)
-{
-    if (!b->marker && b->end - b->p >= 8 && b->n <= 56) {
-        uint64_t w;
-        memcpy(&w, b->p, 8);
-        w = __builtin_bswap64(w);
-        const uint64_t x = ~w;
-        if (!((x - 0x0101010101010101ULL) & ~x & 0x8080808080808080ULL)) {
-            const int nb = (64 - b->n) >> 3;
-            b->acc = nb == 8 ? w : (b->acc << (8 * nb)) | (w >> (64 - 8 * nb));
-            b->p += nb;
-            b->n += 8 * nb;
-            return;
-        }
-    }
-    while (b->n <= 56) {
-        unsigned c = 0;
-        int real = 0;
-        if (!b->marker && b->p < b->end) {
-            c = *b->p;
-            if (c == 0xFF) {
-                if (b->p + 1 < b->end && b->p[1] == 0) { b->p += 2; real = 1; }
-                else { b->marker = 1; c = 0; }
-            } else { b->p++; real = 1; }
-        }
-        b->dry += !real;
-        b->acc = (b->acc << 8) | c;
-        b->n += 8;
-    }
-}
-static inline int bits_get(struct bits *b, int k)
-{
-    if (k == 0) return 0;
-    if (b->n < k) bits_fill(b);
-    b->n -= k;
-    return (int)((b->acc >> b->n) & ((1u << k) - 1));
-}
-static inline int huff_decode(struct bits *b, const struct huff *h)
-{
-    if (b->n < 16) bits_fill(b);
-    unsigned peek = (unsigned)((b->acc >> (b->n - LOOK)) & ((1u << LOOK) - 1));
-    unsigned e = h->look[peek];
-    if (e) { b->n -= (int)(e >> 8); return (int)(e & 0xff); }
-    int code = (int)peek, len = LOOK;
-    while (code > h->maxcode[len]) {
-        if (++len > 16) return -1;
-        code = (int)((b->acc >> (b->n - len)) & ((1u << len) - 1));
-    }
-    b->n -= len;
-    return h->vals[(h->valptr[len] + code - h->mincode[len]) & 255];
-}
-static inline int extend(int v, int t) { return (t && v < (1 << (t - 1))) ? v - (1 << t) + 1 : v; }
+uint64_t ffhip_huff_spec_digest(const struct huff_spec *s)
+{
+    _Static_assert(offsetof(struct huff_spec, vals) == offsetof(struct huff_spec, counts) + 16, "vals follow counts");
+    const uint8_t *p = (const uint8_t *)s + offsetof(struct huff_spec, counts);
+    size_t left = 16 + (size_t)s->n;
+    uint64_t h = 0x9e3779b97f4a7c15ull ^ left;
+    for (; left; p += 8) {
+        uint64_t w = 0;
+        const size_t take = left < 8 ? left : 8;
+        memcpy(&w, p, take);
+        left -= take;
+        h = (h ^ w) * 0xff51afd7ed558ccdull;
+        h ^= h >> 32;
+    }
+    return h;
+}
+
+int ffhip_huff_spec_same(const struct huff_spec *a, const struct huff_spec *b)
+{
+    return a == b || (a->n == b->n && !memcmp(a->counts, b->counts, 16) && !memcmp(a->vals, b->vals, a->n));
+}
 
 static int parse_headers(const uint8_t *f, size_t len, struct jpeg_hdr *j)
 {
@@ -132,7 +110,7 @@
                 i++;
                 if (id > 3 || i + (size_t)64 * (prec + 1) > sl) return FFHIP_EINVAL;
                 for (int k = 0; k < 64; k++, i += prec + 1)
-                    j->quant[id][k_zigzag[k]] = prec ? (uint16_t)((s[i] << 8) | s[i + 1]) : s[i];
+                    j->quant[id][ffhip_zigzag[k]] = prec ? (uint16_t)((s[i] << 8) | s[i + 1]) : s[i];
             }
         } else if (m == 0xC4) {
             size_t i = 0;
@@ -141,7 +119,13 @@
                 int n = 0;
                 for (int k = 0; k < 16; k++) n += s[i + 1 + k];
                 if (tc > 1 || th > 3 || n > 256 || i + 17 + (size_t)n > sl) return FFHIP_EINVAL;
-                if (huff_build(tc ? &j->ac[th] : &j->dc[th], s + i + 1, s + i + 17, n)) return FFHIP_EINVAL;
+                if (huff_spec_check(s + i + 1, n)) return FFHIP_EINVAL;
+                struct huff_spec *t = tc ? &j->ac[th] : &j->dc[th];
+                memcpy(t->counts, s + i + 1, 16);
+                memcpy(t->vals, s + i + 17, (size_t)n);
+                t->n = (uint16_t)n;
+                t->present = 1;
+                t->digest = ffhip_huff_spec_digest(t);
                 i += 17 + (size_t)n;
             }
         } else if (m == 0xC0 || m == 0xC1) {
@@ -192,34 +176,161 @@
 int ffhip_jpeg_parse(const uint8_t *file, size_t len, struct jpeg_hdr *j) { return parse_headers(file, len, j); }
 int ffhip_jpeg_probe_restart(const uint8_t *file, size_t len)
 {
-    struct jpeg_hdr *j = malloc(sizeof *j);
-    if (!j) return -1;
-    const int r = parse_headers(file, len, j) ? -1 : j->restart;
-    free(j);
-    return r;
+    struct jpeg_hdr j;
+    return parse_headers(file, len, &j) ? -1 : j.restart;
 }
 
 int ffhip_jpeg_probe(const uint8_t *file, size_t len, ffhip_jpeg_geom *geom, int *width, int *height)
 {
-    struct jpeg_hdr *j = malloc(sizeof *j);
-    if (!j) return FFHIP_ENOMEM;
-    int rc = file && geom ? parse_headers(file, len, j) : FFHIP_EINVAL;
+    struct jpeg_hdr j;
+    const int rc = file && geom ? parse_headers(file, len, &j) : FFHIP_EINVAL;
     if (rc == FFHIP_OK) {
-        geom->ncomp = j->ncomp;
-        geom->h = j->h[0];
-        geom->v = j->v[0];
-        geom->mcu_cols = (j->width + 8 * j->h[0] - 1) / (8 * j->h[0]);
-        geom->mcu_rows = (j->height + 8 * j->v[0] - 1) / (8 * j->v[0]);
-        for (int c = 0; c < 3; c++) geom->qt_id[c] = c < j->ncomp ? j->tq[c] : 0;
-        if (width) *width = j->width;
-        if (height) *height = j->height;
-    }
-    free(j);
+        geom->ncomp = j.ncomp;
+        geom->h = j.h[0];
+        geom->v = j.v[0];
+        geom->mcu_cols = (j.width + 8 * j.h[0] - 1) / (8 * j.h[0]);
+        geom->mcu_rows = (j.height + 8 * j.v[0] - 1) / (8 * j.v[0]);
+        for (int c = 0; c < 3; c++) geom->qt_id[c] = c < j.ncomp ? j.tq[c] : 0;
+        if (width) *width = j.width;
+        if (height) *height = j.height;
+    }
     return rc;
 }
 
-static int decode_mcus(const struct jpeg_hdr *j, int16_t *const planes[3], struct bits *b, long mcu, long count)
-{
+static const struct huff_spec *table_of(const struct jpeg_hdr *j, int q)
+{
+    const int k = q >> 1 < j->ncomp ? q >> 1 : 0;
+    return q & 1 ? &j->ac[j->ta[k]] : &j->dc[j->td[k]];
+}
+#define RESOLVE_SLOTS 8192
+int ffhip_jpeg_resolve_tables(const struct jpeg_hdr *recs, int n, uint32_t *ids, const struct huff_spec **uniq, size_t cap, size_t *n_uniq)
+{
+    uint16_t slot[RESOLVE_SLOTS];
+    size_t nu = 0;
+    if (cap > FFHIP_HUFF_MAX_TABLES) cap = FFHIP_HUFF_MAX_TABLES;
+    memset(slot, 0, sizeof slot);
+    *n_uniq = 0;
+    for (int i = 0; i < n; i++) {
+        const struct jpeg_hdr *j = &recs[i];
+        uint32_t *id = ids + 6 * (size_t)i;
+        for (int q = 0; q < 6; q++) {
+            const struct huff_spec *t = table_of(j, q);
+            if (q >= 2 && t == table_of(j, q & 1)) { id[q] = id[q & 1]; continue; }
+            if (q >= 4 && t == table_of(j, q - 2)) { id[q] = id[q - 2]; continue; }
+            if (i > 0) {
+                const struct huff_spec *b = uniq[id[q - 6]];
+                if (b->digest == t->digest && ffhip_huff_spec_same(b, t)) { id[q] = id[q - 6]; continue; }
+            }
+            uint32_t at = (uint32_t)(t->digest ^ (t->digest >> 32)) & (RESOLVE_SLOTS - 1), found = 0;
+            for (; slot[at]; at = (at + 1) & (RESOLVE_SLOTS - 1)) {
+                const struct huff_spec *b = uniq[slot[at] - 1];
+                if (b->digest == t->digest && ffhip_huff_spec_same(b, t)) { found = slot[at]; break; }
+            }
+            if (!found) {
+                if (nu == cap) return FFHIP_EINVAL;
+                uniq[nu++] = t;
+                slot[at] = (uint16_t)nu;
+                found = (uint32_t)nu;
+            }
+            id[q] = found - 1;
+        }
+    }
+    *n_uniq = nu;
+    return FFHIP_OK;
+}
+
+#define k_zigzag ffhip_zigzag
+struct bits {
+    const uint8_t *p, *end;
+    uint64_t acc;
+    int n;
+    int marker;
+    int dry;
+};
+
+static inline void bits_fill(struct bits *b)
+{
+    if (!b->marker && b->end - b->p >= 8 && b->n <= 56) {
+        uint64_t w;
+        memcpy(&w, b->p, 8);
+        w = __builtin_bswap64(w);
+        const uint64_t x = ~w;
+        if (!((x - 0x0101010101010101ULL) & ~x & 0x8080808080808080ULL)) {
+            const int nb = (64 - b->n) >> 3;
+            b->acc = nb == 8 ? w : (b->acc << (8 * nb)) | (w >> (64 - 8 * nb));
+            b->p += nb;
+            b->n += 8 * nb;
+            return;
+        }
+    }
+    while (b->n <= 56) {
+        unsigned c = 0;
+        int real = 0;
+        if (!b->marker && b->p < b->end) {
+            c = *b->p;
+            if (c == 0xFF) {
+                if (b->p + 1 < b->end && b->p[1] == 0) { b->p += 2; real = 1; }
+                else { b->marker = 1; c = 0; }
+            } else { b->p++; real = 1; }
+        }
+        b->dry += !real;
+        b->acc = (b->acc << 8) | c;
+        b->n += 8;
+    }
+}
+static inline int bits_get(struct bits *b, int k)
+{
+    if (k == 0) return 0;
+    if (b->n < k) bits_fill(b);
+    b->n -= k;
+    return (int)((b->acc >> b->n) & ((1u << k) - 1));
+}
+static inline int huff_decode(struct bits *b, const struct huff *h)
+{
+    if (b->n < 16) bits_fill(b);
+    unsigned peek = (unsigned)((b->acc >> (b->n - LOOK)) & ((1u << LOOK) - 1));
+    unsigned e = h->look[peek];
+    if (e) { b->n -= (int)(e >> 8); return (int)(e & 0xff); }
+    int code = (int)peek, len = LOOK;
+    while (code > h->maxcode[len]) {
+        if (++len > 16) return -1;
+        code = (int)((b->acc >> (b->n - len)) & ((1u << len) - 1));
+    }
+    b->n -= len;
+    return h->vals[(h->valptr[len] + code - h->mincode[len]) & 255];
+}
+static inline int extend(int v, int t) { return (t && v < (1 << (t - 1))) ? v - (1 << t) + 1 : v; }
+
+struct decode_ctx {
+    struct jpeg_hdr j;
+    struct huff tab[6];
+    const struct huff *dc[3], *ac[3];
+};
+static int build_scan_tables(struct decode_ctx *d)
+{
+    const struct jpeg_hdr *j = &d->j;
+    int used = 0;
+    for (int c = 0; c < j->ncomp; c++) {
+        d->dc[c] = d->ac[c] = NULL;
+        for (int e = 0; e < c; e++) {
+            if (j->td[e] == j->td[c]) d->dc[c] = d->dc[e];
+            if (j->ta[e] == j->ta[c]) d->ac[c] = d->ac[e];
+        }
+        if (!d->dc[c]) {
+            if (ffhip_huff_build(&d->tab[used], &j->dc[j->td[c]])) return FFHIP_EINVAL;
+            d->dc[c] = &d->tab[used++];
+        }
+        if (!d->ac[c]) {
+            if (ffhip_huff_build(&d->tab[used], &j->ac[j->ta[c]])) return FFHIP_EINVAL;
+            d->ac[c] = &d->tab[used++];
+        }
+    }
+    return FFHIP_OK;
+}
+
+static int decode_mcus(const struct decode_ctx *d, int16_t *const planes[3], struct bits *b, long mcu, long count)
+{
+    const struct jpeg_hdr *j = &d->j;
     int pred[3] = {0, 0, 0};
     for (int c = 0; c < j->ncomp; c++) {
         const size_t per = (size_t)j->h[c] * j->v[c] * 64;
@@ -227,7 +338,7 @@
     }
     for (const long end = mcu + count; mcu < end; mcu++) {
         for (int c = 0; c < j->ncomp; c++) {
-            const struct huff *hd = &j->dc[j->td[c]], *ha = &j->ac[j->ta[c]];
+            const struct huff *hd = d->dc[c], *ha = d->ac[c];
             const int nb = j->h[c] * j->v[c];
             for (int k = 0; k < nb; k++) {
                 int16_t *blk = planes[c] + (mcu * nb + k) * 64;
@@ -265,7 +376,7 @@
 }
 
 struct interval_job {
-    const struct jpeg_hdr *j;
+    const struct decode_ctx *d;
     int16_t *planes[3];
     const size_t *seg;
     long n_seg, mcus, first, last;
@@ -274,13 +385,14 @@
 static void *interval_worker(void *arg)
 {
     struct interval_job *w = arg;
+    const struct jpeg_hdr *j = &w->d->j;
     w->rc = FFHIP_OK;
     for (long i = w->first; i < w->last && w->rc == FFHIP_OK; i++) {
-        const uint8_t *p = w->j->scan + w->seg[i];
-        const uint8_t *e = i + 1 < w->n_seg ? w->j->scan + w->seg[i + 1] - 2 : w->j->scan + w->j->scan_len;
+        const uint8_t *p = j->scan + w->seg[i];
+        const uint8_t *e = i + 1 < w->n_seg ? j->scan + w->seg[i + 1] - 2 : j->scan + j->scan_len;
         struct bits b = {p, e, 0, 0, 0, 0};
-        const long mcu = i * w->j->restart, left = w->mcus - mcu;
-        w->rc = decode_mcus(w->j, w->planes, &b, mcu, left < w->j->restart ? left : w->j->restart);
+        const long mcu = i * j->restart, left = w->mcus - mcu;
+        w->rc = decode_mcus(w->d, w->planes, &b, mcu, left < j->restart ? left : j->restart);
     }
     return NULL;
 }
@@ -288,31 +400,34 @@
 int ffhip_jpeg_entropy_decode_mt(const uint8_t *file, size_t len, const ffhip_jpeg_geom *expect, int16_t *coef_y,
                                  int16_t *coef_u, int16_t *coef_v, uint16_t *quant , int n_threads)
 {
-    struct jpeg_hdr *j = malloc(sizeof *j);
-    if (!j) return FFHIP_ENOMEM;
-    int rc = file && coef_y && quant ? parse_headers(file, len, j) : FFHIP_EINVAL;
-    if (rc) { free(j); return rc; }
+    struct decode_ctx *d = malloc(sizeof *d);
+    if (!d) return FFHIP_ENOMEM;
+    struct jpeg_hdr *j = &d->j;
+    int rc = file && coef_y && quant ? ffhip_jpeg_parse(file, len, j) : FFHIP_EINVAL;
+    if (rc) { free(d); return rc; }
     const int mcu_cols = (j->width + 8 * j->h[0] - 1) / (8 * j->h[0]), mcu_rows = (j->height + 8 * j->v[0] - 1) / (8 * j->v[0]);
     if (expect && (expect->mcu_cols != mcu_cols || expect->mcu_rows != mcu_rows || expect->ncomp != j->ncomp ||
-                   expect->h != j->h[0] || expect->v != j->v[0])) { free(j); return FFHIP_EINVAL; }
-    if (j->ncomp == 3 && (!coef_u || !coef_v)) { free(j); return FFHIP_EINVAL; }
+                   expect->h != j->h[0] || expect->v != j->v[0])) { free(d); return FFHIP_EINVAL; }
+    if (j->ncomp == 3 && (!coef_u || !coef_v)) { free(d); return FFHIP_EINVAL; }
+    rc = build_scan_tables(d);
+    if (rc) { free(d); return rc; }
     memcpy(quant, j->quant, sizeof j->quant);
     const long mcus = (long)mcu_cols * mcu_rows;
-    struct interval_job base = {j, {coef_y, coef_u, coef_v}, NULL, 1, mcus, 0, 1, FFHIP_OK};
+    struct interval_job base = {d, {coef_y, coef_u, coef_v}, NULL, 1, mcus, 0, 1, FFHIP_OK};
     if (!j->restart) {
         struct bits b = {j->scan, j->scan + j->scan_len, 0, 0, 0, 0};
-        rc = decode_mcus(j, base.planes, &b, 0, mcus);
-        free(j);
+        rc = decode_mcus(d, base.planes, &b, 0, mcus);
+        free(d);
         return rc;
     }
     const long n_seg = (mcus + j->restart - 1) / j->restart;
     size_t *seg = malloc((size_t)n_seg * sizeof *seg);
-    if (!seg) { free(j); return FFHIP_ENOMEM; }
+    if (!seg) { free(d); return FFHIP_ENOMEM; }
     long found = 1;
     seg[0] = 0;
     for (size_t q = 0; q + 1 < j->scan_len && found < n_seg; q++)
         if (j->scan[q] == 0xFF && j->scan[q + 1] >= 0xD0 && j->scan[q + 1] <= 0xD7) { seg[found++] = q + 2; q++; }
-    if (found != n_seg) { free(seg); free(j); return FFHIP_EINVAL; }
+    if (found != n_seg) { free(seg); free(d); return FFHIP_EINVAL; }
     base.seg = seg;
     base.n_seg = n_seg;
     if (n_threads < 1) n_threads = 1;
@@ -335,7 +450,7 @@
         if (rc == FFHIP_OK) rc = jobs[t].rc;
     }
     free(seg);
-    free(j);
+    free(d);
     return rc;
 }
 
diff --git a/ffpic_amd/csrc/ffhip_entropy_internal.h b/ffpic_amd/csrc/ffhip_entropy_internal.h
--- a/ffpic_amd/csrc/ffhip_entropy_internal.h
+++ b/ffpic_amd/csrc/ffhip_entropy_internal.h
@@ -7,6 +7,8 @@
 #ifdef __cplusplus
 extern "C" {
 #endif
+
+extern const uint8_t ffhip_zigzag[64];
 
 #define LOOK 9
 struct huff {
@@ -18,16 +20,29 @@
     int16_t fast[1 << LOOK];
 };
 
+struct huff_spec {
+    uint64_t digest;
+    uint8_t counts[16];
+    uint8_t vals[256];
+    uint16_t n;
+    uint8_t present;
+};
+
 struct jpeg_hdr {
     int width, height, ncomp, restart;
     int h[3], v[3], tq[3], td[3], ta[3], cid[3];
     uint16_t quant[4][64];
-    struct huff dc[4], ac[4];
+    struct huff_spec dc[4], ac[4];
     const uint8_t *scan;
     size_t scan_len;
 };
 
 int ffhip_jpeg_parse(const uint8_t *file, size_t len, struct jpeg_hdr *j);
+int ffhip_huff_build(struct huff *h, const struct huff_spec *s);
+uint64_t ffhip_huff_spec_digest(const struct huff_spec *s);
+int ffhip_huff_spec_same(const struct huff_spec *a, const struct huff_spec *b);
+#define FFHIP_HUFF_MAX_TABLES 4095
+int ffhip_jpeg_resolve_tables(const struct jpeg_hdr *recs, int n, uint32_t *ids, const struct huff_spec **uniq, size_t cap, size_t *n_uniq);
 int ffhip_jpeg_probe_restart(const uint8_t *file, size_t len);
 
 #ifdef __cplusplus
diff --git a/ffpic_amd/csrc/ffhip_huff_gpu.hip b/ffpic_amd/csrc/ffhip_huff_gpu.hip
--- a/ffpic_amd/csrc/ffhip_huff_gpu.hip
+++ b/ffpic_amd/csrc/ffhip_huff_gpu.hip
@@ -9,6 +9,7 @@
 #include <stdlib.h>
 #include <string.h>
 
+#include <algorithm>
 #include <vector>
 #include <memory>
 #include <new>
@@ -273,12 +274,14 @@
 extern "C" int ffhip_jpeg_lut_test(const uint8_t *file, size_t len, int which, uint16_t *out)
 {
     if (!file || !out || which < 0 || which > 7) return FFHIP_EINVAL;
-    std::unique_ptr<struct jpeg_hdr> j(new (std::nothrow) struct jpeg_hdr);
-    if (!j) return FFHIP_ENOMEM;
-    if (ffhip_jpeg_parse(file, len, j.get())) return FFHIP_EINVAL;
-    const struct huff &h = which < 4 ? j->dc[which] : j->ac[which - 4];
-    if (!h.present) return FFHIP_EINVAL;
-    build_lut(h, out);
+    struct jpeg_hdr j;
+    if (ffhip_jpeg_parse(file, len, &j)) return FFHIP_EINVAL;
+    const struct huff_spec &sp = which < 4 ? j.dc[which] : j.ac[which - 4];
+    if (!sp.present) return FFHIP_EINVAL;
+    std::unique_ptr<struct huff> h(new (std::nothrow) struct huff);
+    if (!h) return FFHIP_ENOMEM;
+    if (ffhip_huff_build(h.get(), &sp)) return FFHIP_EINVAL;
+    build_lut(*h, out);
     return FFHIP_OK;
 }
 
@@ -352,10 +355,11 @@
     const FfhipHuffThen *then;
     std::vector<uint32_t> pic_mcus, mcu_base;
     struct jpeg_hdr *hdr;
-    std::vector<std::vector<uint32_t>> segs, raws;
+    uint32_t *segs, *raws;
     uint32_t sub_bits;
     std::vector<HuffImage> images;
-    std::vector<const struct huff *> uniq;
+    std::vector<const struct huff_spec *> uniq;
+    std::vector<uint32_t> tab_ids;
     size_t scan_total, seg_total;
     HuffLayout L;
     uint8_t *stage, *dev;
@@ -394,8 +398,7 @@
 {
     c.hdr = ffhip_huff_hdr_records((size_t)c.n);
     if (!c.hdr) return FFHIP_ENOMEM;
-    c.segs.resize((size_t)c.n);
-    c.raws.resize((size_t)c.n);
+    c.images.resize((size_t)c.n);
     ffhip_parallel_for(c.n, c.n_threads, [&c](int i) {
         struct jpeg_hdr &j = c.hdr[(size_t)i];
         c.status[i] = ffhip_jpeg_parse(c.files[i], c.lens[i], &j);
@@ -409,55 +412,59 @@
             return;
         }
         if (!j.restart) j.restart = (int)mcus;
-        c.segs[(size_t)i].assign((size_t)((mcus + j.restart - 1) / j.restart) + 1, 0u);
-        c.raws[(size_t)i].assign(c.segs[(size_t)i].size(), 0u);
-    });
-    return huff_first_status(c);
-}
-bool huff_choose_subsequences(HuffCall &c)
-{
-    const char *sy = FFHIP_ENV("FFHIP_JPEG_SYNC");
-    unsigned long long batch_bits = 0, n_int = 0;
-    for (int i = 0; i < c.n; i++) batch_bits += 8ull * c.hdr[(size_t)i].scan_len;
-    c.sub_bits = sync_sub_bits(batch_bits, (unsigned long long)c.mcu_base[(size_t)c.n]);
-    if (sy && (sy[0] == '0' || sy[0] == '1')) return sy[0] == '1';
-    for (int i = 0; i < c.n; i++) n_int += c.segs[(size_t)i].size() - 1;
-    return batch_bits > 2ull * c.sub_bits * n_int;
-}
-uint32_t huff_table_id(std::vector<const struct huff *> &uniq, const struct huff *t)
-{
-    for (size_t u = uniq.size(); u-- > 0;)
-        if (uniq[u] == t || !memcmp(&uniq[u]->maxcode, &t->maxcode, offsetof(struct huff, fast) - offsetof(struct huff, maxcode))) return (uint32_t)u;
-    uniq.push_back(t);
-    return (uint32_t)(uniq.size() - 1);
-}
-int huff_lay_out(HuffCall &c)
-{
-    c.images.resize((size_t)c.n);
-    c.scan_total = c.seg_total = 0;
-    for (int i = 0; i < c.n; i++) {
-        const struct jpeg_hdr &j = c.hdr[(size_t)i];
         HuffImage &im = c.images[(size_t)i];
-        im.scan_off = (uint32_t)c.scan_total;
         im.scan_len = (uint32_t)j.scan_len;
         im.restart = (uint32_t)j.restart;
         im.mcus = c.pic_mcus[(size_t)i];
         im.mcu_base = c.mcu_base[(size_t)i];
         im.ncomp = (uint32_t)j.ncomp;
-        im.seg_base = (uint32_t)c.seg_total;
-        im.n_seg = (uint32_t)c.segs[(size_t)i].size() - 1;
+        im.n_seg = (uint32_t)((mcus + (size_t)j.restart - 1) / (size_t)j.restart);
+        for (int k = 0; k < 3; k++) im.nb[k] = k < j.ncomp ? (uint32_t)(j.h[k] * j.v[k]) : 0;
+    });
+    const int rc = huff_first_status(c);
+    if (rc) return rc;
+    size_t at = 0;
+    for (int i = 0; i < c.n; i++) {
+        c.images[(size_t)i].seg_base = (uint32_t)at;
+        at += (size_t)c.images[(size_t)i].n_seg + 1;
+        if (at > 0x7fffffffu) return FFHIP_EINVAL;
+    }
+    c.seg_total = at - (size_t)c.n;
+    c.segs = ffhip_huff_interval_lists(2 * at);
+    if (!c.segs) return FFHIP_ENOMEM;
+    c.raws = c.segs + at;
+    return FFHIP_OK;
+}
+bool huff_choose_subsequences(HuffCall &c)
+{
+    const char *sy = FFHIP_ENV("FFHIP_JPEG_SYNC");
+    unsigned long long batch_bits = 0, n_int = 0;
+    for (int i = 0; i < c.n; i++) batch_bits += 8ull * c.images[(size_t)i].scan_len;
+    c.sub_bits = sync_sub_bits(batch_bits, (unsigned long long)c.mcu_base[(size_t)c.n]);
+    if (sy && (sy[0] == '0' || sy[0] == '1')) return sy[0] == '1';
+    n_int = c.seg_total;
+    return batch_bits > 2ull * c.sub_bits * n_int;
+}
+int huff_lay_out(HuffCall &c)
+{
+    c.scan_total = 0;
+    size_t n_uniq = 0;
+    c.tab_ids.resize(6 * (size_t)c.n);
+    c.uniq.resize(std::min<size_t>(6 * (size_t)c.n, FFHIP_HUFF_MAX_TABLES));
+    const int too_many = ffhip_jpeg_resolve_tables(c.hdr, c.n, c.tab_ids.data(), c.uniq.data(), c.uniq.size(), &n_uniq);
+    c.uniq.resize(n_uniq);
+    for (int i = 0; i < c.n; i++) {
+        HuffImage &im = c.images[(size_t)i];
+        im.scan_off = (uint32_t)c.scan_total;
         for (int k = 0; k < 3; k++) {
-            im.nb[k] = k < j.ncomp ? (uint32_t)(j.h[k] * j.v[k]) : 0;
-            im.tab_dc[k] = huff_table_id(c.uniq, &j.dc[k < j.ncomp ? j.td[k] : j.td[0]]);
-            im.tab_ac[k] = huff_table_id(c.uniq, &j.ac[k < j.ncomp ? j.ta[k] : j.ta[0]]);
-        }
-        c.scan_total += (j.scan_len + 8 * (size_t)im.n_seg + 64 + 15) & ~(size_t)15;
-        c.seg_total += im.n_seg;
-        im.seg_base += (uint32_t)i;
+            im.tab_dc[k] = c.tab_ids[6 * (size_t)i + 2 * (size_t)k];
+            im.tab_ac[k] = c.tab_ids[6 * (size_t)i + 2 * (size_t)k + 1];
+        }
+        c.scan_total += ((size_t)im.scan_len + 8 * (size_t)im.n_seg + 64 + 15) & ~(size_t)15;
         if (c.scan_total > 0x7fffffffu) return FFHIP_EINVAL;
     }
     if (!ffhip_have_device()) return FFHIP_ENODEV;
-    if (c.uniq.size() > 4095) return FFHIP_EINVAL;
+    if (too_many) return FFHIP_EINVAL;
     c.L = huff_layout(c.scan_total, c.uniq.size(), (size_t)c.n, c.seg_total);
     c.stage = ffhip_pinned_scratch(SCRATCH_HUFF, c.st, c.L.total + 64);
     if (!c.stage) return FFHIP_ENOMEM;
@@ -481,9 +488,11 @@
         const struct jpeg_hdr &j = c.hdr[(size_t)i];
         const HuffImage &im = c.images[(size_t)i];
         uint8_t *dst = c.stage + im.scan_off;
-        std::vector<uint32_t> &sgv = c.segs[(size_t)i];
+        uint32_t *sgv = c.segs + im.seg_base, *raw = c.raws + im.seg_base;
         size_t off = 0;
-        if (stage_scan(dst, j.scan, j.scan + j.scan_len, sgv.data(), im.n_seg, &off, c.raws[(size_t)i].data()) != im.n_seg) c.status[i] = FFHIP_EINVAL;
+        memset(sgv, 0, ((size_t)im.n_seg + 1) * 4);
+        memset(raw, 0, ((size_t)im.n_seg + 1) * 4);
+        if (stage_scan(dst, j.scan, j.scan + j.scan_len, sgv, im.n_seg, &off, raw) != im.n_seg) c.status[i] = FFHIP_EINVAL;
         memset(dst + off, 0, 16);
         sgv[im.n_seg] = (uint32_t)off;
         if (!lists) return;
@@ -505,9 +514,12 @@
 {
     const HuffTime Ta = huff_now();
     memset(c.stage + c.scan_total, 0, 16);
-    ffhip_parallel_for((int)c.uniq.size(), c.n_threads, [&c](int u) {
-        ((struct huff *)(c.stage + c.L.o_tabs))[u] = *c.uniq[(size_t)u];
-        build_lut(*c.uniq[(size_t)u], (uint16_t *)(c.stage + c.L.o_l12) + (size_t)u * LUT_WORDS);
+    struct huff *built = ffhip_huff_built_tables(c.uniq.size());
+    if (!built) return FFHIP_ENOMEM;
+    ffhip_parallel_for((int)c.uniq.size(), c.n_threads, [&c, built](int u) {
+        (void)ffhip_huff_build(&built[u], c.uniq[(size_t)u]);
+        ((struct huff *)(c.stage + c.L.o_tabs))[u] = built[u];
+        build_lut(built[u], (uint16_t *)(c.stage + c.L.o_l12) + (size_t)u * LUT_WORDS);
     });
     memcpy(c.stage + c.L.o_img, c.images.data(), c.images.size() * sizeof(HuffImage));
     memset(c.stage + c.L.o_status, 0, (size_t)c.n * 4);
@@ -604,14 +616,14 @@
     segs.clear();
     for (int i = lo; i < hi; i++) {
         const HuffImage &im = c.images[(size_t)i];
-        const std::vector<uint32_t> &sgv = c.segs[(size_t)i];
+        const uint32_t *sgv = c.segs + im.seg_base, *raw = c.raws + im.seg_base;
         if (c.status[i]) return c.status[i];
         for (uint32_t k = 0; k < im.n_seg; k++) {
             SyncSeg sg;
             sg.pic = (uint32_t)(i - lo);
             sg.scan_off = im.scan_off + sgv[k];
             sg.clean_len = sgv[k + 1] - sgv[k];
-            sg.raw_len = c.raws[(size_t)i][k];
+            sg.raw_len = raw[k];
             sg.mcu0 = (uint32_t)((size_t)(c.mcu_base[(size_t)i] - c.mcu_base[(size_t)lo]) + (size_t)k * im.restart);
             const size_t left = im.mcus - (size_t)k * im.restart;
             sg.mcus = (uint32_t)(left < im.restart ? left : im.restart);
diff --git a/ffpic_amd/csrc/ffhip_internal.h b/ffpic_amd/csrc/ffhip_internal.h
--- a/ffpic_amd/csrc/ffhip_internal.h
+++ b/ffpic_amd/csrc/ffhip_internal.h
@@ -211,6 +211,8 @@
 void ffhip_pipeline_release(void);
 int ffhip_vp8_side_by_side_retry(void *stream);
 struct jpeg_hdr *ffhip_huff_hdr_records(size_t n);
+struct huff *ffhip_huff_built_tables(size_t n);
+uint32_t *ffhip_huff_interval_lists(size_t n);
 
 struct FfhipSide { void *stream, *fork, *join, *mid; };
 extern "C" int ffhip_side_stream_get(FfhipSide *out);
diff --git a/ffpic_amd/csrc/ffhip_state.hip b/ffpic_amd/csrc/ffhip_state.hip
--- a/ffpic_amd/csrc/ffhip_state.hip
+++ b/ffpic_amd/csrc/ffhip_state.hip
@@ -134,6 +134,10 @@
     std::map<int, ThreadSet> sets;
     std::unique_ptr<struct jpeg_hdr[]> hdr;
     size_t hdr_cap = 0;
+    std::unique_ptr<struct huff[]> tabs;
+    size_t tabs_cap = 0;
+    std::unique_ptr<uint32_t[]> ivals;
+    size_t ivals_cap = 0;
     ThreadState() { std::lock_guard<std::mutex> l(g_ffhip_state_mu); g_threads.push_back(this); }
     ~ThreadState()
     {
@@ -179,16 +183,20 @@
     return FFHIP_OK;
 }
 
-struct jpeg_hdr *ffhip_huff_hdr_records(size_t n)
-{
-    ThreadState &t = this_thread();
+namespace {
+template <class T> T *kept(std::unique_ptr<T[]> &buf, size_t &cap, size_t n)
+{
     std::lock_guard<std::mutex> l(g_ffhip_state_mu);
-    if (n > t.hdr_cap) {
-        t.hdr.reset(new (std::nothrow) struct jpeg_hdr[n + n / 4]);
-        t.hdr_cap = t.hdr ? n + n / 4 : 0;
-    }
-    return t.hdr.get();
-}
+    if (n > cap) {
+        buf.reset(new (std::nothrow) T[n + n / 4]);
+        cap = buf ? n + n / 4 : 0;
+    }
+    return buf.get();
+}
+}
+struct jpeg_hdr *ffhip_huff_hdr_records(size_t n) { ThreadState &t = this_thread(); return kept(t.hdr, t.hdr_cap, n); }
+struct huff *ffhip_huff_built_tables(size_t n) { ThreadState &t = this_thread(); return kept(t.tabs, t.tabs_cap, n); }
+uint32_t *ffhip_huff_interval_lists(size_t n) { ThreadState &t = this_thread(); return kept(t.ivals, t.ivals_cap, n); }
 
 void ffhip_state_release(void)
 {
@@ -200,6 +208,8 @@
         for (auto &e : t->sets) e.second.release();
         t->sets.clear();
         t->hdr.reset();
-        t->hdr_cap = 0;
-    }
-}
+        t->tabs.reset();
+        t->ivals.reset();
+        t->hdr_cap = t->tabs_cap = t->ivals_cap = 0;
+    }
+}
```

Measured after the change: 859,900 Mpixels/s (median of 2 runs). Within noise of the previous version (+1.0%).
